# ibm-granite/dolomite-engine

Hardware: AMD Instinct MI355X
Metric: tokens/sec/node GPTDolomite-3B bf16 seq4096 padding-free (higher is better)
Workload: dtype bf16; 1 GPU; gptdolomite-3b-bf16-seq4096-paddingfree-pretrain; model=GPTDolomite-3B, global_batch=16, seq_len=4096, parallelism=dp1

## Files before the change

dolomite_engine_amd/csrc/attention.hip:

```cpp

#include "common.h"

typedef __bf16 bf16x8 __attribute__((ext_vector_type(8)));
typedef float f32x4 __attribute__((ext_vector_type(4)));

#define MFMA16(a, b, c) __builtin_amdgcn_mfma_f32_16x16x32_bf16((a), (b), (c), 0, 0, 0)

#define DOL_LOG2E 1.44269504088896340736f
#define DOL_LN2 0.69314718055994530942f

#define PI23(q) (((q) & ~12) | ((((q) >> 2) & 1) << 3) | ((((q) >> 3) & 1) << 2))

typedef __bf16 bf16x4 __attribute__((ext_vector_type(4)));


__device__ __forceinline__ bf16x8 lds_tr16_bfrag(const __bf16* img, int rowbase, int S, int d0, int lane) {
    const int g8 = (lane >> 4) * 8;
    const int jj = (lane >> 2) & 3;
    const int cc = (lane & 3) * 4;
    unsigned a0 = (unsigned)(size_t)(img + PI23(rowbase + g8 + jj) * S + d0 + cc);
    unsigned a1 = (unsigned)(size_t)(img + PI23(rowbase + g8 + 4 + jj) * S + d0 + cc);
    bf16x4 lo, hi;
    asm volatile(
        "ds_read_b64_tr_b16 %0, %2\n\t"
        "ds_read_b64_tr_b16 %1, %3\n\t"
        "s_waitcnt lgkmcnt(0)"
        : "=&v"(lo), "=&v"(hi)
        : "v"(a0), "v"(a1)
        : "memory");
    bf16x8 out;
#pragma unroll
    for (int t = 0; t < 4; ++t) { out[t] = lo[t]; out[4 + t] = hi[t]; }
    return out;
}


template <int OFF>
__device__ __forceinline__ void tr16_issue(unsigned a0, unsigned a1, bf16x4& lo, bf16x4& hi) {
    asm volatile(
        "ds_read_b64_tr_b16 %0, %2 offset:%c4\n\t"
        "ds_read_b64_tr_b16 %1, %3 offset:%c4"
        : "=&v"(lo), "=&v"(hi)
        : "v"(a0), "v"(a1), "i"(OFF)
        : "memory");
}

template <int N>
__device__ __forceinline__ void lgkm_wait2(bf16x4& a, bf16x4& b) {
    asm volatile("s_waitcnt lgkmcnt(%c2)" : "+v"(a), "+v"(b) : "i"(N));
}
template <int N>
__device__ __forceinline__ void lgkm_wait4(bf16x4& a, bf16x4& b, bf16x4& c, bf16x4& d) {
    asm volatile("s_waitcnt lgkmcnt(%c4)" : "+v"(a), "+v"(b), "+v"(c), "+v"(d) : "i"(N));
}
template <int N>
__device__ __forceinline__ void lgkm_wait8(bf16x4& a, bf16x4& b, bf16x4& c, bf16x4& d,
                                           bf16x4& e, bf16x4& f, bf16x4& g, bf16x4& h) {
    asm volatile("s_waitcnt lgkmcnt(%c8)"
                 : "+v"(a), "+v"(b), "+v"(c), "+v"(d), "+v"(e), "+v"(f), "+v"(g), "+v"(h)
                 : "i"(N));
}

__device__ __forceinline__ bf16x8 tr16_join8(bf16x4 lo, bf16x4 hi) {
    bf16x8 out;
#pragma unroll
    for (int t = 0; t < 4; ++t) { out[t] = lo[t]; out[4 + t] = hi[t]; }
    return out;
}

__device__ __forceinline__ void lgkm_drain2x8(bf16x8& a, bf16x8& b) {
    asm volatile("s_waitcnt lgkmcnt(0)" : "+v"(a), "+v"(b));
}
__device__ __forceinline__ void lgkm_drain4x8(bf16x8& a, bf16x8& b, bf16x8& c, bf16x8& d) {
    asm volatile("s_waitcnt lgkmcnt(0)" : "+v"(a), "+v"(b), "+v"(c), "+v"(d));
}

__device__ __forceinline__ bf16x8 load_bf16x8_guard(const __bf16* p, int d0, int D, bool valid) {
    const __bf16* q = (d0 < D) ? p : (p - d0);
    bool ok = valid && (d0 < D);
    bf16x8 r = *(const bf16x8*)q;
#pragma unroll
    for (int e = 0; e < 8; ++e) r[e] = ok ? r[e] : (__bf16)0.f;
    return r;
}

__device__ __forceinline__ float qwave_reduce_max(float v) {
    v = fmaxf(v, dpp_ror_f32<8>(v));
    v = fmaxf(v, dpp_ror_f32<4>(v));
    v = fmaxf(v, dpp_ror_f32<2>(v));
    v = fmaxf(v, dpp_ror_f32<1>(v));
    return v;
}
__device__ __forceinline__ float qwave_reduce_sum(float v) {
    v += dpp_ror_f32<8>(v);
    v += dpp_ror_f32<4>(v);
    v += dpp_ror_f32<2>(v);
    v += dpp_ror_f32<1>(v);
    return v;
}


__device__ __forceinline__ void xcd_remap_tile_bh(int& tile, int& b, int& h) {
    const int ntile = gridDim.x, nb = gridDim.y, nh = gridDim.z;
    const int64_t nbh = (int64_t)nb * nh;
    if (nbh % 8 != 0) return;
    int64_t raw = blockIdx.x + (int64_t)ntile * (blockIdx.y + (int64_t)nb * blockIdx.z);
    int xcd = (int)(raw % 8);
    int64_t idx = raw / 8;
    int64_t pair_local = idx / ntile;
    tile = (int)(idx % ntile);
    int64_t pair = pair_local * 8 + xcd;
    b = (int)(pair % nb);
    h = (int)(pair / nb);
}

#define DOL_DROP_CQ 0x9E3779B1u
#define DOL_DROP_CK 0x85EBCA77u
#define DOL_DROP_CH 0xC2B2AE3Du
#define DOL_DROP_M1 0x7FEB352Du
#define DOL_DROP_M2 0x846CA68Bu

__device__ __forceinline__ uint32_t drop_mix32(uint32_t x) {
    x ^= x >> 16;
    x *= DOL_DROP_M1;
    x ^= x >> 15;
    x *= DOL_DROP_M2;
    x ^= x >> 16;
    return x;
}
__device__ __forceinline__ uint32_t drop_head_word(uint32_t seed_hi, uint32_t h) {
    return drop_mix32(seed_hi ^ (h * DOL_DROP_CH));
}
__device__ __forceinline__ uint32_t drop_row_word(uint32_t seed_lo, uint32_t t_q) {
    return drop_mix32(seed_lo ^ (t_q * DOL_DROP_CQ));
}
__device__ __forceinline__ uint32_t drop_col_word(uint32_t head_word, uint32_t t_k) {
    return drop_mix32(head_word ^ (t_k * DOL_DROP_CK));
}
__device__ __forceinline__ bool drop_keep_words(uint32_t rw, uint32_t cw, uint32_t thr) {
    uint32_t x = rw ^ cw;
    x ^= x >> 16;
    x *= DOL_DROP_M1;
    x ^= x >> 15;
    x *= DOL_DROP_M2;
    return x >= thr;
}
__device__ __forceinline__ bool drop_keep(uint32_t seed_lo, uint32_t seed_hi, uint32_t h,
                                          uint32_t t_q, uint32_t t_k, uint32_t thr) {
    return drop_keep_words(drop_row_word(seed_lo, t_q),
                           drop_col_word(drop_head_word(seed_hi, h), t_k), thr);
}

static inline uint32_t drop_threshold(float p_drop) {
    return (uint32_t)((double)p_drop * 4294967296.0);
}
static inline bool drop_p_valid(float p_drop) { return p_drop >= 0.f && p_drop < 1.f; }


template <int DPAD, bool DROPOUT>
__global__ void __launch_bounds__(512, 4) fa_fwd_kernel(
    const __bf16* __restrict__ q, const __bf16* __restrict__ k, const __bf16* __restrict__ v,
    __bf16* __restrict__ o, float* __restrict__ lse,
    const int32_t* __restrict__ cu, int H, int Hkv, int D, int G,
    int64_t q_ts, int64_t q_gs, int64_t k_ts, int64_t k_hs, int64_t v_ts, int64_t v_hs,
    int64_t o_ts, int64_t T_total, float scale,
    uint32_t seed_lo, uint32_t seed_hi, uint32_t drop_thr, float drop_rp) {
    constexpr int KCH = DPAD / 32;
    constexpr int DCH = DPAD / 16;
    constexpr int SK = DPAD + 16;
    constexpr int SV = 64 + 8;

    int tile_id = blockIdx.x, b = blockIdx.y, h = blockIdx.z;
    xcd_remap_tile_bh(tile_id, b, h);
    const int s0 = __builtin_amdgcn_readfirstlane(cu[b]);
    const int L = __builtin_amdgcn_readfirstlane(cu[b + 1]) - s0;
    const int ntile_seq = (L + 127) / 128;
    if (tile_id >= ntile_seq) return;
    const int qs = (ntile_seq - 1 - tile_id) * 128;

    const int lane = threadIdx.x & 63;
    const int wave = threadIdx.x >> 6;
    const int lr = lane & 15;
    const int lg = lane >> 4;

    constexpr int NBUF = 1;
    extern __shared__ char smem_raw[];
    __bf16* Klds = (__bf16*)smem_raw;
    __bf16* Vlds = Klds + NBUF * 64 * SK;
    __bf16* Plds = Vlds + NBUF * 64 * SK;
    __bf16* Pw = Plds + wave * 16 * SV;

    const int kvh = h / G;
    const int64_t q_hoff = (int64_t)(h / G) * q_gs + (int64_t)(h % G) * D;

    const int qrow = qs + wave * 16 + lr;
    const bool qvalid = qrow < L;
    bf16x8 qf[KCH];
#pragma unroll
    for (int kc = 0; kc < KCH; ++kc) {
        int d0 = kc * 32 + lg * 8;
        const __bf16* p = q + (int64_t)(s0 + (qvalid ? qrow : 0)) * q_ts + q_hoff + d0;
        qf[kc] = load_bf16x8_guard(p, d0, D, qvalid);
    }

    float m_run[4], l_run[4];
    f32x4 o_acc[DCH];
#pragma unroll
    for (int r = 0; r < 4; ++r) { m_run[r] = -INFINITY; l_run[r] = 0.f; }
#pragma unroll
    for (int dc = 0; dc < DCH; ++dc) o_acc[dc] = {0.f, 0.f, 0.f, 0.f};

    uint32_t drop_rw[4];
    uint32_t drop_hw = 0;
    if constexpr (DROPOUT) {
        drop_hw = drop_head_word(seed_hi, (uint32_t)h);
#pragma unroll
        for (int r = 0; r < 4; ++r)
            drop_rw[r] = drop_row_word(seed_lo, (uint32_t)(s0 + qs + wave * 16 + lg * 4 + r));
    }

    const int tr_jj = (lane >> 2) & 3;
    const int tr_g8 = (lane >> 4) * 8;
    const int tr_cc = (lane & 3) * 4;
    const unsigned aV0 = (unsigned)(size_t)(Vlds + PI23(tr_g8 + tr_jj) * SK + tr_cc);
    const unsigned aV1 = (unsigned)(size_t)(Vlds + PI23(tr_g8 + 4 + tr_jj) * SK + tr_cc);

    const int kend = min(L, qs + 128);
    const int ntiles = (kend + 63) / 64;

    if (D < DPAD) {
        for (int pidx = threadIdx.x; pidx < 64 * (DPAD - D) / 8; pidx += 512) {
            int key = pidx / ((DPAD - D) / 8);
            int d0 = D + (pidx % ((DPAD - D) / 8)) * 8;
            bf16x8 z = {};
            *(bf16x8*)&Klds[key * SK + d0] = z;
            *(bf16x8*)&Vlds[PI23(key) * SK + d0] = z;
        }
    }

    int st_koff[2], st_voff[2];
    int st_klds[2], st_vlds[2];
#pragma unroll
    for (int j = 0; j < 2; ++j) {
        int pidx = (int)threadIdx.x + j * 512;
        int pp = pidx < 64 * D / 8 ? pidx : 0;
        int key = pp / (D / 8);
        int d0 = (pp % (D / 8)) * 8;
        st_koff[j] = (int)(key * k_ts + kvh * k_hs) + d0;
        st_voff[j] = (int)(key * v_ts + kvh * v_hs) + d0;
        st_klds[j] = key * SK + d0;
        st_vlds[j] = PI23(key) * SK + d0;
    }

    if (__builtin_amdgcn_readfirstlane(threadIdx.x) >= 256) __builtin_amdgcn_s_setprio(1);

    constexpr int PIECES = 64 * DPAD / 8;

    auto stage_direct = [&](int ks_, __bf16* Kw, __bf16* Vw) {
        if (ks_ + 64 <= kend) {
            const int64_t disp = (int64_t)(s0 + ks_);
#pragma unroll
            for (int j = 0; j < 2; ++j) {
                if ((int)threadIdx.x + j * 512 < 64 * D / 8) {
                    *(bf16x8*)&Kw[st_klds[j]] = *(const bf16x8*)(k + disp * k_ts + st_koff[j]);
                    *(bf16x8*)&Vw[st_vlds[j]] = *(const bf16x8*)(v + disp * v_ts + st_voff[j]);
                }
            }
        } else {
            for (int pidx = threadIdx.x; pidx < PIECES; pidx += 512) {
                int key = pidx / (DPAD / 8);
                int d0 = (pidx % (DPAD / 8)) * 8;
                bool kv_valid = (ks_ + key) < kend;
                const __bf16* kp = k + (int64_t)(s0 + (kv_valid ? ks_ + key : 0)) * k_ts + (int64_t)kvh * k_hs + d0;
                *(bf16x8*)&Kw[key * SK + d0] = load_bf16x8_guard(kp, d0, D, kv_valid);
                const __bf16* vp = v + (int64_t)(s0 + (kv_valid ? ks_ + key : 0)) * v_ts + (int64_t)kvh * v_hs + d0;
                *(bf16x8*)&Vw[PI23(key) * SK + d0] = load_bf16x8_guard(vp, d0, D, kv_valid);
            }
        }
    };

    auto compute_tile = [&](const __bf16* Kb, unsigned aV0c, unsigned aV1c, int ks) {
        f32x4 sc[4];
#pragma unroll
        for (int cb = 0; cb < 4; ++cb) {
            sc[cb] = {0.f, 0.f, 0.f, 0.f};
#pragma unroll
            for (int kc = 0; kc < KCH; ++kc) {
                bf16x8 kf = *(const bf16x8*)&Kb[(cb * 16 + lr) * SK + kc * 32 + lg * 8];
                sc[cb] = MFMA16(qf[kc], kf, sc[cb]);
            }
        }

        const float scale2 = scale * DOL_LOG2E;
        const bool edge_tile =
            !((ks + 63 <= qs + wave * 16) && (ks + 64 <= kend) && (qs + wave * 16 + 16 <= L));
        uint32_t drop_cw[4];
        if constexpr (DROPOUT) {
#pragma unroll
            for (int cb = 0; cb < 4; ++cb)
                drop_cw[cb] = drop_col_word(drop_hw, (uint32_t)(s0 + ks + cb * 16 + lr));
        }
#pragma unroll
        for (int r = 0; r < 4; ++r) {
            float pv[4];
#pragma unroll
            for (int cb = 0; cb < 4; ++cb) pv[cb] = sc[cb][r] * scale2;
            if (__builtin_amdgcn_readfirstlane(edge_tile ? 1 : 0)) {
                const int qpos = qs + wave * 16 + lg * 4 + r;
#pragma unroll
                for (int cb = 0; cb < 4; ++cb) {
                    const int kpos = ks + cb * 16 + lr;
                    if (kpos > qpos || kpos >= kend || qpos >= L) pv[cb] = -INFINITY;
                }
            }
            float rowmax = fmaxf(fmaxf(pv[0], pv[1]), fmaxf(pv[2], pv[3]));
            rowmax = qwave_reduce_max(rowmax);
            float mnew = fmaxf(m_run[r], rowmax);
            if (mnew == -INFINITY) mnew = 0.f;
            float alpha = exp2f(m_run[r] - mnew);
            float rsum = 0.f;
#pragma unroll
            for (int cb = 0; cb < 4; ++cb) {
                float e = exp2f(pv[cb] - mnew);
                float ek = e;
                if constexpr (DROPOUT)
                    ek = drop_keep_words(drop_rw[r], drop_cw[cb], drop_thr) ? e : 0.f;
                Pw[(lg * 4 + r) * SV + cb * 16 + lr] = (__bf16)ek;
                rsum += e;
            }
            rsum = qwave_reduce_sum(rsum);
            l_run[r] = l_run[r] * alpha + rsum;
            m_run[r] = mnew;
#pragma unroll
            for (int dc = 0; dc < DCH; ++dc) o_acc[dc][r] *= alpha;
        }

        {
            bf16x8 pf0 = *(const bf16x8*)&Pw[lr * SV + lg * 8];
            bf16x8 pf1 = *(const bf16x8*)&Pw[lr * SV + 32 + lg * 8];
            lgkm_drain2x8(pf0, pf1);
            __builtin_amdgcn_sched_barrier(0);
            bf16x4 vlo[3], vhi[3];
            tr16_issue<0>(aV0c, aV1c, vlo[0], vhi[0]);
            tr16_issue<((1 / DCH) * 32 * SK + (1 % DCH) * 16) * 2>(aV0c, aV1c, vlo[1], vhi[1]);
#define FWD_PV_STEP(i)                                                                                  \
    if constexpr ((i) < 2 * DCH) {                                                                      \
        constexpr int kc2_ = (i) / DCH, dc_ = (i) % DCH;                                                \
        if constexpr ((i) + 2 < 2 * DCH) {                                                              \
            constexpr int kn_ = ((i) + 2) / DCH, dn_ = ((i) + 2) % DCH;                                 \
            tr16_issue<(kn_ * 32 * SK + dn_ * 16) * 2>(aV0c, aV1c, vlo[((i) + 2) % 3], vhi[((i) + 2) % 3]); \
            lgkm_wait2<4>(vlo[(i) % 3], vhi[(i) % 3]);                                                  \
        } else if constexpr ((i) + 1 < 2 * DCH) {                                                       \
            lgkm_wait2<2>(vlo[(i) % 3], vhi[(i) % 3]);                                                  \
        } else {                                                                                        \
            lgkm_wait2<0>(vlo[(i) % 3], vhi[(i) % 3]);                                                  \
        }                                                                                               \
        o_acc[dc_] = MFMA16(kc2_ ? pf1 : pf0, tr16_join8(vlo[(i) % 3], vhi[(i) % 3]), o_acc[dc_]);      \
    }
            FWD_PV_STEP(0) FWD_PV_STEP(1) FWD_PV_STEP(2) FWD_PV_STEP(3)
            FWD_PV_STEP(4) FWD_PV_STEP(5) FWD_PV_STEP(6) FWD_PV_STEP(7)
            FWD_PV_STEP(8) FWD_PV_STEP(9) FWD_PV_STEP(10) FWD_PV_STEP(11)
            FWD_PV_STEP(12) FWD_PV_STEP(13) FWD_PV_STEP(14) FWD_PV_STEP(15)
#undef FWD_PV_STEP
            __builtin_amdgcn_sched_barrier(0);
        }
    };

    if constexpr (NBUF == 2) {
        constexpr int CH = (64 * SK * 2) / 1024;
        constexpr int NC = (2 * CH + 7) / 8;
        auto rsrcK = __builtin_amdgcn_make_buffer_rsrc(
            (void*)(k + (int64_t)s0 * k_ts + (int64_t)kvh * k_hs), 0,
            (unsigned)(((int64_t)(L - 1) * k_ts + D) * 2), 0);
        auto rsrcV = __builtin_amdgcn_make_buffer_rsrc(
            (void*)(v + (int64_t)s0 * v_ts + (int64_t)kvh * v_hs), 0,
            (unsigned)(((int64_t)(L - 1) * v_ts + D) * 2), 0);
        unsigned choff[NC];
        bool ch_is_v[NC];
#pragma unroll
        for (int i = 0; i < NC; ++i) {
            int c = wave + i * 8;
            bool isv = c >= CH;
            int cc = isv ? c - CH : c;
            int e0 = cc * 512 + lane * 8;
            int row = e0 / SK;
            int col = e0 % SK;
            int key = isv ? PI23(row) : row;
            int64_t ts = isv ? v_ts : k_ts;
            unsigned off = (unsigned)((key * ts + col) * 2);
            if (col >= D || c >= 2 * CH) off = 0x40000000u;
            choff[i] = off;
            ch_is_v[i] = isv;
        }
        const unsigned kstep2 = (unsigned)(k_ts * 2) * 64u;
        const unsigned vstep2 = (unsigned)(v_ts * 2) * 64u;

        auto stage_dma = [&](int kt_, int buf_) {
            __bf16* Kb = Klds + buf_ * 64 * SK;
            __bf16* Vb = Vlds + buf_ * 64 * SK;
#pragma unroll
            for (int i = 0; i < NC; ++i) {
                int c = wave + i * 8;
                if (c >= 2 * CH) break;
                bool isv = ch_is_v[i];
                int cc = isv ? c - CH : c;
                char* ldsp = (char*)(isv ? Vb : Kb) + cc * 1024;
                unsigned vo = choff[i] + (unsigned)kt_ * (isv ? vstep2 : kstep2);
                __builtin_amdgcn_raw_ptr_buffer_load_lds(
                    isv ? rsrcV : rsrcK,
                    (__attribute__((address_space(3))) void*)ldsp, 16, vo, 0, 0, 0);
            }
        };

        stage_dma(0, 0);
        asm volatile("s_waitcnt vmcnt(0)" ::: "memory");
        __syncthreads();
        for (int kt = 0; kt < ntiles; ++kt) {
            const int cur = kt & 1;
            if (kt + 1 < ntiles) stage_dma(kt + 1, cur ^ 1);
            compute_tile(Klds + cur * 64 * SK,
                         aV0 + (unsigned)(cur * 64 * SK * 2),
                         aV1 + (unsigned)(cur * 64 * SK * 2), kt * 64);
            asm volatile("s_waitcnt vmcnt(0)" ::: "memory");
            __syncthreads();
        }
    } else {
        for (int kt = 0; kt < ntiles; ++kt) {
            stage_direct(kt * 64, Klds, Vlds);
            __syncthreads();
            compute_tile(Klds, aV0, aV1, kt * 64);
            __syncthreads();
        }
    }

    float inv_l[4];
#pragma unroll
    for (int r = 0; r < 4; ++r) {
        inv_l[r] = (l_run[r] > 0.f) ? 1.f / l_run[r] : 0.f;
        if constexpr (DROPOUT) inv_l[r] *= drop_rp;
        const int qpos = qs + wave * 16 + lg * 4 + r;
        if (lr == 0 && qpos < L)
            lse[(int64_t)h * T_total + s0 + qpos] = (m_run[r] + log2f(l_run[r])) * DOL_LN2;
    }
#pragma unroll
    for (int dc = 0; dc < DCH; ++dc) {
#pragma unroll
        for (int r = 0; r < 4; ++r) {
            const int qpos = qs + wave * 16 + lg * 4 + r;
            const int d = dc * 16 + lr;
            if (qpos < L && d < D)
                o[(int64_t)(s0 + qpos) * o_ts + (int64_t)h * D + d] = (__bf16)(o_acc[dc][r] * inv_l[r]);
        }
    }
}

template <int DPAD, bool DROPOUT>
static int launch_fa_fwd(hipStream_t stream, const __bf16* q, const __bf16* k, const __bf16* v,
                         __bf16* o, float* lse, const int32_t* cu, int batch, int64_t T,
                         int H, int Hkv, int D, int G,
                         int64_t q_ts, int64_t q_gs, int64_t k_ts, int64_t k_hs,
                         int64_t v_ts, int64_t v_hs, int max_tiles, float scale,
                         float p_drop, uint64_t seed) {
    dim3 grid(max_tiles, batch, H), block(512);
    size_t shmem = ((size_t)(DPAD <= 96 ? 2 : 1) * 64 * (DPAD + 16) * 2 + 8 * 16 * 72) * sizeof(__bf16);
    hipLaunchKernelGGL((fa_fwd_kernel<DPAD, DROPOUT>), grid, block, shmem, stream,
                       q, k, v, o, lse, cu, H, Hkv, D, G,
                       q_ts, q_gs, k_ts, k_hs, v_ts, v_hs, (int64_t)H * D, T, scale,
                       (uint32_t)seed, (uint32_t)(seed >> 32), drop_threshold(p_drop),
                       1.f / (1.f - p_drop));
    return dol_last_error();
}

static int fa_varlen_fwd_dispatch(dolomite_stream_t stream,
                                  const void* q, const void* k, const void* v,
                                  void* o, float* lse,
                                  const int32_t* cu_seqlens, int batch, int max_seqlen, int64_t T,
                                  int H, int Hkv, int D, int G,
                                  int64_t q_tstride, int64_t q_gstride,
                                  int64_t k_tstride, int64_t k_hstride,
                                  int64_t v_tstride, int64_t v_hstride,
                                  float scale, int dtype, float p_drop, uint64_t seed) {
    if (dtype != DOLOMITE_BF16) return 9010;
    if (D > 128) return 9011;
    int max_tiles = (max_seqlen + 127) / 128;
    hipStream_t s = (hipStream_t)stream;
#define CASE(DP, DROP)                                                                               \
    return launch_fa_fwd<DP, DROP>(s, (const __bf16*)q, (const __bf16*)k, (const __bf16*)v,          \
                                   (__bf16*)o, lse, cu_seqlens, batch, T, H, Hkv, D, G, q_tstride,   \
                                   q_gstride, k_tstride, k_hstride, v_tstride, v_hstride, max_tiles, \
                                   scale, p_drop, seed)
    if (p_drop > 0.f) {
        if (D <= 32) CASE(32, true);
        if (D <= 64) CASE(64, true);
        if (D <= 96) CASE(96, true);
        CASE(128, true);
    }
    if (D <= 32) CASE(32, false);
    if (D <= 64) CASE(64, false);
    if (D <= 96) CASE(96, false);
    CASE(128, false);
#undef CASE
}

extern "C" int dolomite_fa_varlen_fwd(dolomite_stream_t stream,
                                      const void* q, const void* k, const void* v,
                                      void* o, float* lse,
                                      const int32_t* cu_seqlens, int batch, int max_seqlen, int64_t T,
                                      int H, int Hkv, int D, int G,
                                      int64_t q_tstride, int64_t q_gstride,
                                      int64_t k_tstride, int64_t k_hstride,
                                      int64_t v_tstride, int64_t v_hstride,
                                      float scale, int dtype) {
    return fa_varlen_fwd_dispatch(stream, q, k, v, o, lse, cu_seqlens, batch, max_seqlen, T,
                                  H, Hkv, D, G, q_tstride, q_gstride, k_tstride, k_hstride,
                                  v_tstride, v_hstride, scale, dtype, 0.f, 0);
}

extern "C" int dolomite_fa_varlen_fwd_dropout(dolomite_stream_t stream,
                                              const void* q, const void* k, const void* v,
                                              void* o, float* lse,
                                              const int32_t* cu_seqlens, int batch, int max_seqlen, int64_t T,
                                              int H, int Hkv, int D, int G,
                                              int64_t q_tstride, int64_t q_gstride,
                                              int64_t k_tstride, int64_t k_hstride,
                                              int64_t v_tstride, int64_t v_hstride,
                                              float scale, int dtype, float p_drop, uint64_t seed) {
    if (!drop_p_valid(p_drop)) return 9013;
    return fa_varlen_fwd_dispatch(stream, q, k, v, o, lse, cu_seqlens, batch, max_seqlen, T,
                                  H, Hkv, D, G, q_tstride, q_gstride, k_tstride, k_hstride,
                                  v_tstride, v_hstride, scale, dtype, p_drop, seed);
}


template <typename T>
__global__ void __launch_bounds__(256) fa_bwd_preprocess_kernel(
    const T* __restrict__ o, const T* __restrict__ dout, float* __restrict__ delta,
    int64_t T_total, int H, int D, int64_t o_ts, int64_t do_ts) {
    int64_t row = ((int64_t)blockIdx.x * 4) + (threadIdx.x >> 6);
    int lane = threadIdx.x & 63;
    if (row >= T_total * H) return;
    int64_t t = row / H;
    int h = (int)(row % H);
    const T* op = o + t * o_ts + (int64_t)h * D;
    const T* dp = dout + t * do_ts + (int64_t)h * D;
    float acc = 0.f;
    for (int d = lane * 2; d + 1 < D; d += 128) {
        float o0[2], d0[2];
        VecIO<T, 2>::load(op + d, o0);
        VecIO<T, 2>::load(dp + d, d0);
        acc += o0[0] * d0[0] + o0[1] * d0[1];
    }
    if (D & 1) {
        int d = D - 1;
        if (lane == 0) acc += load_as_f32(op + d) * load_as_f32(dp + d);
    }
    acc = wave_reduce_sum(acc);
    if (lane == 0) delta[(int64_t)h * T_total + t] = acc;
}

__global__ void __launch_bounds__(256) fa_bwd_preprocess_tiled(
    const __bf16* __restrict__ o, const __bf16* __restrict__ dout, float* __restrict__ delta,
    int64_t T_total, int H, int D, int TOK) {
    extern __shared__ float part[];
    const int64_t hd = (int64_t)H * D;
    const int64_t base = (int64_t)blockIdx.x * TOK * hd;
    const int64_t total = T_total * hd;
    const int np = (int)(TOK * hd / 8);
#pragma unroll 4
    for (int p = threadIdx.x; p < np; p += 256) {
        int64_t flat = base + (int64_t)p * 8;
        float acc = 0.f;
        if (flat + 8 <= total) {
            bf16x8 ov = *(const bf16x8*)(o + flat);
            bf16x8 dv = *(const bf16x8*)(dout + flat);
#pragma unroll
            for (int e = 0; e < 8; ++e) acc += (float)ov[e] * (float)dv[e];
        }
        part[p] = acc;
    }
    __syncthreads();
    const int slots = TOK * H;
    const int dp8 = D / 8;
    for (int s = threadIdx.x; s < slots; s += 256) {
        float a = 0.f;
        const float* ps = &part[s * dp8];
        for (int i = 0; i < dp8; ++i) a += ps[i];
        int tl = s / H, h = s - tl * H;
        int64_t t = (int64_t)blockIdx.x * TOK + tl;
        if (t < T_total) delta[(int64_t)h * T_total + t] = a;
    }
}

extern "C" int dolomite_fa_bwd_preprocess(dolomite_stream_t stream,
                                          const void* o, const void* dout, float* delta,
                                          int64_t T, int H, int D,
                                          int64_t o_tstride, int64_t do_tstride, int dtype) {
    const int64_t hd = (int64_t)H * D;
    int TOK = 16;
    while (TOK > 1 && TOK * hd * 4 / 8 > 65536) TOK /= 2;
    if (dtype == DOLOMITE_BF16 && D % 8 == 0 && o_tstride == hd && do_tstride == hd && T > 0 &&
        TOK * hd * 4 / 8 <= 65536) {
        dim3 grid((uint32_t)((T + TOK - 1) / TOK)), block(256);
        size_t shmem = (size_t)(TOK * hd / 8) * sizeof(float);
        hipLaunchKernelGGL((fa_bwd_preprocess_tiled), grid, block, shmem, (hipStream_t)stream,
                           (const __bf16*)o, (const __bf16*)dout, delta, T, H, D, TOK);
        return dol_last_error();
    }
    int64_t rows = T * H;
    dim3 grid((uint32_t)((rows + 3) / 4)), block(256);
    if (dtype == DOLOMITE_BF16)
        hipLaunchKernelGGL((fa_bwd_preprocess_kernel<uint16_t>), grid, block, 0, (hipStream_t)stream,
                           (const uint16_t*)o, (const uint16_t*)dout, delta, T, H, D, o_tstride, do_tstride);
    else
        hipLaunchKernelGGL((fa_bwd_preprocess_kernel<float>), grid, block, 0, (hipStream_t)stream,
                           (const float*)o, (const float*)dout, delta, T, H, D, o_tstride, do_tstride);
    return dol_last_error();
}



template <int DPAD, bool DROPOUT>
__global__ void __launch_bounds__(512, DPAD <= 96 ? 4 : 2) fa_bwd_dkv_kernel(
    const __bf16* __restrict__ q, const __bf16* __restrict__ k, const __bf16* __restrict__ v,
    const __bf16* __restrict__ dout, const float* __restrict__ lse, const float* __restrict__ delta,
    float* __restrict__ dk_acc, float* __restrict__ dv_acc,
    const int32_t* __restrict__ cu, int H, int Hkv, int D, int G,
    int64_t q_ts, int64_t q_gs, int64_t k_ts, int64_t k_hs, int64_t v_ts, int64_t v_hs,
    int64_t do_ts, int64_t T_total, float scale,
    uint32_t seed_lo, uint32_t seed_hi, uint32_t drop_thr, float drop_rp) {
    constexpr int KCH = DPAD / 32;
    constexpr int DCH = DPAD / 16;

    int tile_id = blockIdx.x, b = blockIdx.y, h = blockIdx.z;
    xcd_remap_tile_bh(tile_id, b, h);
    const int kvh = h / G;
    const int s0 = __builtin_amdgcn_readfirstlane(cu[b]);
    const int L = __builtin_amdgcn_readfirstlane(cu[b + 1]) - s0;
    const int ks = tile_id * 128;
    if (ks >= L) return;

    const int lane = threadIdx.x & 63;
    const int wave = threadIdx.x >> 6;
    const int lr = lane & 15;
    const int lg = lane >> 4;

    constexpr int SQ = DPAD + 16;
    constexpr int STS = 128 + 4;
    extern __shared__ char smem_raw[];
    __bf16* Qlds = (__bf16*)smem_raw;
    __bf16* dOl = Qlds + 64 * SQ;
    __bf16* dSTl = dOl + 64 * SQ;
    __bf16* PTl = dSTl + 64 * STS;

    const int kend = min(L, ks + 128);

    const int krow = ks + wave * 16 + lr;
    const bool kvalid = krow < kend;
    bf16x8 kfr[KCH], vfr[KCH];
#pragma unroll
    for (int kc = 0; kc < KCH; ++kc) {
        int d0 = kc * 32 + lg * 8;
        const __bf16* kp = k + (int64_t)(s0 + (kvalid ? krow : 0)) * k_ts + (int64_t)kvh * k_hs + d0;
        kfr[kc] = load_bf16x8_guard(kp, d0, D, kvalid);
        const __bf16* vp = v + (int64_t)(s0 + (kvalid ? krow : 0)) * v_ts + (int64_t)kvh * v_hs + d0;
        vfr[kc] = load_bf16x8_guard(vp, d0, D, kvalid);
    }

    f32x4 dvr[DCH], dkr[DCH];
#pragma unroll
    for (int dc = 0; dc < DCH; ++dc) {
        dvr[dc] = {0.f, 0.f, 0.f, 0.f};
        dkr[dc] = {0.f, 0.f, 0.f, 0.f};
    }

    uint32_t drop_cw[4];
    if constexpr (DROPOUT) {
        const uint32_t drop_hw = drop_head_word(seed_hi, (uint32_t)h);
#pragma unroll
        for (int r = 0; r < 4; ++r)
            drop_cw[r] = drop_col_word(drop_hw, (uint32_t)(s0 + ks + wave * 16 + lg * 4 + r));
    }

    const int tr_jj = (lane >> 2) & 3;
    const int tr_g8 = (lane >> 4) * 8;
    const int tr_cc = (lane & 3) * 4;
    const unsigned aQ0 = (unsigned)(size_t)(Qlds + PI23(tr_g8 + tr_jj) * SQ + tr_cc);
    const unsigned aQ1 = (unsigned)(size_t)(Qlds + PI23(tr_g8 + 4 + tr_jj) * SQ + tr_cc);
    const unsigned aDS0 = (unsigned)(size_t)(dSTl + PI23(tr_g8 + tr_jj) * STS + wave * 16 + tr_cc);
    const unsigned aDS1 = (unsigned)(size_t)(dSTl + PI23(tr_g8 + 4 + tr_jj) * STS + wave * 16 + tr_cc);
    constexpr int DO_IMM = 64 * SQ * 2;
    constexpr int PT_IMM = 64 * STS * 2;
    static_assert(DO_IMM + 32 * SQ * 2 + 16 * 2 < 65536, "ds offset range");
    static_assert(PT_IMM + 32 * STS * 2 + 16 * 2 < 65536, "ds offset range");

    if (__builtin_amdgcn_readfirstlane(threadIdx.x) >= 256) __builtin_amdgcn_s_setprio(1);

    const int qt0 = ks / 64;
    const int nqt = (L + 63) / 64;
    const int64_t q_hoff = (int64_t)(h / G) * q_gs + (int64_t)(h % G) * D;
    const int64_t do_hoff = (int64_t)h * D;

    if (D < DPAD) {
        for (int pidx = threadIdx.x; pidx < 64 * (DPAD - D) / 8; pidx += 512) {
            int qq = pidx / ((DPAD - D) / 8);
            int d0 = D + (pidx % ((DPAD - D) / 8)) * 8;
            bf16x8 z = {};
            *(bf16x8*)&Qlds[PI23(qq) * SQ + d0] = z;
            *(bf16x8*)&dOl[PI23(qq) * SQ + d0] = z;
        }
    }

    const unsigned st_magic = (1u << 22) / (unsigned)(D / 8) + 1;
    for (int qt = qt0; qt < nqt; ++qt) {
        const int qs = qt * 64;
        __syncthreads();
        {
            const int pieces = 64 * DPAD / 8;
            if (qs + 64 <= L) {
                for (int pidx = threadIdx.x; pidx < 64 * D / 8; pidx += 512) {
                    int qq = (int)(((unsigned)pidx * st_magic) >> 22);
                    int d0 = (pidx - qq * (D / 8)) * 8;
                    *(bf16x8*)&Qlds[PI23(qq) * SQ + d0] =
                        *(const bf16x8*)(q + (int64_t)(s0 + qs + qq) * q_ts + q_hoff + d0);
                    *(bf16x8*)&dOl[PI23(qq) * SQ + d0] =
                        *(const bf16x8*)(dout + (int64_t)(s0 + qs + qq) * do_ts + do_hoff + d0);
                }
            } else {
                for (int pidx = threadIdx.x; pidx < pieces; pidx += 512) {
                    int qq = pidx / (DPAD / 8);
                    int d0 = (pidx % (DPAD / 8)) * 8;
                    bool valid = (qs + qq) < L;
                    const __bf16* qp = q + (int64_t)(s0 + (valid ? qs + qq : 0)) * q_ts + q_hoff + d0;
                    *(bf16x8*)&Qlds[PI23(qq) * SQ + d0] = load_bf16x8_guard(qp, d0, D, valid);
                    const __bf16* dp = dout + (int64_t)(s0 + (valid ? qs + qq : 0)) * do_ts + do_hoff + d0;
                    *(bf16x8*)&dOl[PI23(qq) * SQ + d0] = load_bf16x8_guard(dp, d0, D, valid);
                }
            }
        }
        __syncthreads();

        const bool full_tile = (ks + wave * 16 + 16 <= qs + 1) && (kend == ks + 64) && (qs + 64 <= L);
#pragma unroll
        for (int cb = 0; cb < 4; ++cb) {
            f32x4 st = {0.f, 0.f, 0.f, 0.f};
            f32x4 dpt = {0.f, 0.f, 0.f, 0.f};
#pragma unroll
            for (int kc = 0; kc < KCH; ++kc) {
                int d0 = kc * 32 + lg * 8;
                bf16x8 qb = *(const bf16x8*)&Qlds[(cb * 16 + PI23(lr)) * SQ + d0];
                st = MFMA16(kfr[kc], qb, st);
                bf16x8 db = *(const bf16x8*)&dOl[(cb * 16 + PI23(lr)) * SQ + d0];
                dpt = MFMA16(vfr[kc], db, dpt);
            }
            const int qpos = qs + cb * 16 + lr;
            const bool qok = qpos < L;
            float lsev = qok ? lse[(int64_t)h * T_total + s0 + qpos] * DOL_LOG2E : 0.f;
            float delv = qok ? delta[(int64_t)h * T_total + s0 + qpos] : 0.f;
            bf16x4 pvv, dsv;
            uint32_t drop_rw = 0;
            if constexpr (DROPOUT) drop_rw = drop_row_word(seed_lo, (uint32_t)(s0 + qpos));
            if (__builtin_amdgcn_readfirstlane(full_tile ? 1 : 0)) {
#pragma unroll
                for (int r = 0; r < 4; ++r) {
                    float pv = exp2f(st[r] * (scale * DOL_LOG2E) - lsev);
                    if constexpr (DROPOUT) {
                        const bool keep = drop_keep_words(drop_rw, drop_cw[r], drop_thr);
                        pvv[r] = (__bf16)(keep ? pv : 0.f);
                        dsv[r] = (__bf16)(pv * ((keep ? dpt[r] * drop_rp : 0.f) - delv) * scale);
                    } else {
                        pvv[r] = (__bf16)pv;
                        dsv[r] = (__bf16)(pv * (dpt[r] - delv) * scale);
                    }
                }
            } else {
#pragma unroll
                for (int r = 0; r < 4; ++r) {
                    const int kpos = ks + wave * 16 + lg * 4 + r;
                    bool ok = qok && kpos < kend && kpos <= qpos;
                    float pv = ok ? exp2f(st[r] * (scale * DOL_LOG2E) - lsev) : 0.f;
                    if constexpr (DROPOUT) {
                        const bool keep = drop_keep_words(drop_rw, drop_cw[r], drop_thr);
                        float ds = ok ? pv * ((keep ? dpt[r] * drop_rp : 0.f) - delv) * scale : 0.f;
                        pvv[r] = (__bf16)(keep ? pv : 0.f);
                        dsv[r] = (__bf16)ds;
                    } else {
                        float ds = ok ? pv * (dpt[r] - delv) * scale : 0.f;
                        pvv[r] = (__bf16)pv;
                        dsv[r] = (__bf16)ds;
                    }
                }
            }
            const int srow = PI23(cb * 16 + lr) * STS + wave * 16 + lg * 4;
            *(bf16x4*)&PTl[srow] = pvv;
            *(bf16x4*)&dSTl[srow] = dsv;
        }

        {
            asm volatile("s_waitcnt lgkmcnt(0)" ::: "memory");
            __builtin_amdgcn_sched_barrier(0);
            bf16x4 a_lo[2], a_hi[2];
            tr16_issue<PT_IMM>(aDS0, aDS1, a_lo[0], a_hi[0]);
            tr16_issue<PT_IMM + 32 * STS * 2>(aDS0, aDS1, a_lo[1], a_hi[1]);
            bf16x4 blo[3], bhi[3];
            tr16_issue<DO_IMM>(aQ0, aQ1, blo[0], bhi[0]);
            tr16_issue<DO_IMM + ((1 / DCH) * 32 * SQ + (1 % DCH) * 16) * 2>(aQ0, aQ1, blo[1], bhi[1]);
            lgkm_wait4<4>(a_lo[0], a_hi[0], a_lo[1], a_hi[1]);
            bf16x8 af0 = tr16_join8(a_lo[0], a_hi[0]);
            bf16x8 af1 = tr16_join8(a_lo[1], a_hi[1]);
#define DKV_HALF(i, IMM, ACC, AF0, AF1)                                                                 \
    if constexpr ((i) < 2 * DCH) {                                                                      \
        constexpr int kc2_ = (i) / DCH, dc_ = (i) % DCH;                                                \
        if constexpr ((i) + 2 < 2 * DCH) {                                                              \
            constexpr int kn_ = ((i) + 2) / DCH, dn_ = ((i) + 2) % DCH;                                 \
            tr16_issue<(kn_ * 32 * SQ + dn_ * 16) * 2 + (IMM)>(aQ0, aQ1, blo[((i) + 2) % 3], bhi[((i) + 2) % 3]); \
            lgkm_wait2<4>(blo[(i) % 3], bhi[(i) % 3]);                                                  \
        } else if constexpr ((i) + 1 < 2 * DCH) {                                                       \
            lgkm_wait2<2>(blo[(i) % 3], bhi[(i) % 3]);                                                  \
        } else {                                                                                        \
            lgkm_wait2<0>(blo[(i) % 3], bhi[(i) % 3]);                                                  \
        }                                                                                               \
        ACC[dc_] = MFMA16(kc2_ ? (AF1) : (AF0), tr16_join8(blo[(i) % 3], bhi[(i) % 3]), ACC[dc_]);      \
    }
#define DKV_A(i) DKV_HALF(i, DO_IMM, dvr, af0, af1)
            DKV_A(0) DKV_A(1) DKV_A(2) DKV_A(3)
            DKV_A(4) DKV_A(5) DKV_A(6) DKV_A(7)
            DKV_A(8) DKV_A(9) DKV_A(10) DKV_A(11)
            DKV_A(12) DKV_A(13) DKV_A(14) DKV_A(15)
#undef DKV_A
            tr16_issue<0>(aDS0, aDS1, a_lo[0], a_hi[0]);
            tr16_issue<32 * STS * 2>(aDS0, aDS1, a_lo[1], a_hi[1]);
            tr16_issue<0>(aQ0, aQ1, blo[0], bhi[0]);
            tr16_issue<((1 / DCH) * 32 * SQ + (1 % DCH) * 16) * 2>(aQ0, aQ1, blo[1], bhi[1]);
            lgkm_wait4<4>(a_lo[0], a_hi[0], a_lo[1], a_hi[1]);
            af0 = tr16_join8(a_lo[0], a_hi[0]);
            af1 = tr16_join8(a_lo[1], a_hi[1]);
#define DKV_B(i) DKV_HALF(i, 0, dkr, af0, af1)
            DKV_B(0) DKV_B(1) DKV_B(2) DKV_B(3)
            DKV_B(4) DKV_B(5) DKV_B(6) DKV_B(7)
            DKV_B(8) DKV_B(9) DKV_B(10) DKV_B(11)
            DKV_B(12) DKV_B(13) DKV_B(14) DKV_B(15)
#undef DKV_B
#undef DKV_HALF
            __builtin_amdgcn_sched_barrier(0);
        }
    }

#pragma unroll
    for (int dc = 0; dc < DCH; ++dc) {
#pragma unroll
        for (int r = 0; r < 4; ++r) {
            const int kpos = ks + wave * 16 + lg * 4 + r;
            const int d = dc * 16 + lr;
            if (kpos < kend && d < D) {
                int64_t idx = ((int64_t)(s0 + kpos) * H + h) * D + d;
                __builtin_nontemporal_store(dkr[dc][r], &dk_acc[idx]);
                if constexpr (DROPOUT)
                    __builtin_nontemporal_store(dvr[dc][r] * drop_rp, &dv_acc[idx]);
                else
                    __builtin_nontemporal_store(dvr[dc][r], &dv_acc[idx]);
            }
        }
    }
}

template <int DPAD, bool DROPOUT>
__global__ void __launch_bounds__(512, (DROPOUT && DPAD > 96) ? 2 : 4) fa_bwd_dq_kernel(
    const __bf16* __restrict__ q, const __bf16* __restrict__ k, const __bf16* __restrict__ v,
    const __bf16* __restrict__ dout, const float* __restrict__ lse, const float* __restrict__ delta,
    __bf16* __restrict__ dqkv_q,
    const int32_t* __restrict__ cu, int H, int Hkv, int D, int G,
    int64_t q_ts, int64_t q_gs, int64_t k_ts, int64_t k_hs, int64_t v_ts, int64_t v_hs,
    int64_t do_ts, int64_t T_total, float scale,
    uint32_t seed_lo, uint32_t seed_hi, uint32_t drop_thr, float drop_rp) {
    constexpr int KCH = DPAD / 32;
    constexpr int DCH = DPAD / 16;
    constexpr int ST = 64 + 8;

    int tile_id = blockIdx.x, b = blockIdx.y, h = blockIdx.z;
    xcd_remap_tile_bh(tile_id, b, h);
    const int kvh = h / G;
    const int s0 = __builtin_amdgcn_readfirstlane(cu[b]);
    const int L = __builtin_amdgcn_readfirstlane(cu[b + 1]) - s0;
    const int ntile_seq = (L + 127) / 128;
    if (tile_id >= ntile_seq) return;
    const int qs = (ntile_seq - 1 - tile_id) * 128;

    const int lane = threadIdx.x & 63;
    const int wave = threadIdx.x >> 6;
    const int lr = lane & 15;
    const int lg = lane >> 4;

    constexpr int SQ = DPAD + 16;
    extern __shared__ char smem_raw[];
    __bf16* Klds = (__bf16*)smem_raw;
    __bf16* Vlds = Klds + 64 * SQ;
    __bf16* dSl = Vlds + 64 * SQ;
    __bf16* dSw = dSl + wave * 16 * ST;

    const int64_t q_hoff = (int64_t)(h / G) * q_gs + (int64_t)(h % G) * D;
    const int64_t do_hoff = (int64_t)h * D;

    const int tr_jj = (lane >> 2) & 3;
    const int tr_g8 = (lane >> 4) * 8;
    const int tr_cc = (lane & 3) * 4;
    const unsigned aK0 = (unsigned)(size_t)(Klds + PI23(tr_g8 + tr_jj) * SQ + tr_cc);
    const unsigned aK1 = (unsigned)(size_t)(Klds + PI23(tr_g8 + 4 + tr_jj) * SQ + tr_cc);

    const int qrow = qs + wave * 16 + lr;
    const bool qvalid = qrow < L;
    bf16x8 qfr[KCH], dfr[KCH];
#pragma unroll
    for (int kc = 0; kc < KCH; ++kc) {
        int d0 = kc * 32 + lg * 8;
        const __bf16* qp = q + (int64_t)(s0 + (qvalid ? qrow : 0)) * q_ts + q_hoff + d0;
        qfr[kc] = load_bf16x8_guard(qp, d0, D, qvalid);
        const __bf16* dp = dout + (int64_t)(s0 + (qvalid ? qrow : 0)) * do_ts + do_hoff + d0;
        dfr[kc] = load_bf16x8_guard(dp, d0, D, qvalid);
    }

    float lsev[4], delv[4];
#pragma unroll
    for (int r = 0; r < 4; ++r) {
        const int qp_ = qs + wave * 16 + lg * 4 + r;
        bool ok = qp_ < L;
        lsev[r] = ok ? lse[(int64_t)h * T_total + s0 + qp_] * DOL_LOG2E : 0.f;
        delv[r] = ok ? delta[(int64_t)h * T_total + s0 + qp_] : 0.f;
    }

    f32x4 dq[DCH];
#pragma unroll
    for (int dc = 0; dc < DCH; ++dc) dq[dc] = {0.f, 0.f, 0.f, 0.f};

    uint32_t drop_rw[4];
    uint32_t drop_hw = 0;
    if constexpr (DROPOUT) {
        drop_hw = drop_head_word(seed_hi, (uint32_t)h);
#pragma unroll
        for (int r = 0; r < 4; ++r)
            drop_rw[r] = drop_row_word(seed_lo, (uint32_t)(s0 + qs + wave * 16 + lg * 4 + r));
    }

    if (D < DPAD) {
        for (int pidx = threadIdx.x; pidx < 64 * (DPAD - D) / 8; pidx += 512) {
            int key = pidx / ((DPAD - D) / 8);
            int d0 = D + (pidx % ((DPAD - D) / 8)) * 8;
            bf16x8 z = {};
            *(bf16x8*)&Klds[PI23(key) * SQ + d0] = z;
            *(bf16x8*)&Vlds[key * SQ + d0] = z;
        }
    }

    int st_koff[2], st_voff[2];
    int st_klds[2], st_vlds[2];
#pragma unroll
    for (int j = 0; j < 2; ++j) {
        int pidx = (int)threadIdx.x + j * 512;
        int pp = pidx < 64 * D / 8 ? pidx : 0;
        int key = pp / (D / 8);
        int d0 = (pp % (D / 8)) * 8;
        st_koff[j] = (int)(key * k_ts + kvh * k_hs) + d0;
        st_voff[j] = (int)(key * v_ts + kvh * v_hs) + d0;
        st_klds[j] = PI23(key) * SQ + d0;
        st_vlds[j] = key * SQ + d0;
    }

    const int kend_total = min(L, qs + 128);
    const int nkt = (kend_total + 63) / 64;

    if (__builtin_amdgcn_readfirstlane(threadIdx.x) >= 256) __builtin_amdgcn_s_setprio(1);

    for (int kt = 0; kt < nkt; ++kt) {
        const int ks = kt * 64;
        __syncthreads();
        {
            const int pieces = 64 * DPAD / 8;
            if (ks + 64 <= kend_total) {
                const int64_t disp = (int64_t)(s0 + ks);
#pragma unroll
                for (int j = 0; j < 2; ++j) {
                    if ((int)threadIdx.x + j * 512 < 64 * D / 8) {
                        *(bf16x8*)&Klds[st_klds[j]] = *(const bf16x8*)(k + disp * k_ts + st_koff[j]);
                        *(bf16x8*)&Vlds[st_vlds[j]] = *(const bf16x8*)(v + disp * v_ts + st_voff[j]);
                    }
                }
            } else {
                for (int pidx = threadIdx.x; pidx < pieces; pidx += 512) {
                    int key = pidx / (DPAD / 8);
                    int d0 = (pidx % (DPAD / 8)) * 8;
                    bool valid = (ks + key) < kend_total;
                    const __bf16* kp = k + (int64_t)(s0 + (valid ? ks + key : 0)) * k_ts + (int64_t)kvh * k_hs + d0;
                    *(bf16x8*)&Klds[PI23(key) * SQ + d0] = load_bf16x8_guard(kp, d0, D, valid);
                    const __bf16* vp = v + (int64_t)(s0 + (valid ? ks + key : 0)) * v_ts + (int64_t)kvh * v_hs + d0;
                    *(bf16x8*)&Vlds[key * SQ + d0] = load_bf16x8_guard(vp, d0, D, valid);
                }
            }
        }
        __syncthreads();

        const bool full_tile = (ks + 64 <= qs + wave * 16 + 1) && (ks + 64 <= kend_total) && (qs + wave * 16 + 16 <= L);
#pragma unroll
        for (int cb = 0; cb < 4; ++cb) {
            f32x4 sc = {0.f, 0.f, 0.f, 0.f};
            f32x4 dp = {0.f, 0.f, 0.f, 0.f};
#pragma unroll
            for (int kc = 0; kc < KCH; ++kc) {
                int d0 = kc * 32 + lg * 8;
                bf16x8 kb = *(const bf16x8*)&Klds[(cb * 16 + PI23(lr)) * SQ + d0];
                sc = MFMA16(qfr[kc], kb, sc);
                bf16x8 vb = *(const bf16x8*)&Vlds[(cb * 16 + lr) * SQ + d0];
                dp = MFMA16(dfr[kc], vb, dp);
            }
            uint32_t drop_cw = 0;
            if constexpr (DROPOUT) drop_cw = drop_col_word(drop_hw, (uint32_t)(s0 + ks + cb * 16 + lr));
            if (__builtin_amdgcn_readfirstlane(full_tile ? 1 : 0)) {
#pragma unroll
                for (int r = 0; r < 4; ++r) {
                    float pv = exp2f(sc[r] * (scale * DOL_LOG2E) - lsev[r]);
                    float dpm = dp[r];
                    if constexpr (DROPOUT)
                        dpm = drop_keep_words(drop_rw[r], drop_cw, drop_thr) ? dp[r] * drop_rp : 0.f;
                    dSw[(lg * 4 + r) * ST + cb * 16 + lr] = (__bf16)(pv * (dpm - delv[r]) * scale);
                }
            } else {
#pragma unroll
                for (int r = 0; r < 4; ++r) {
                    const int qpos = qs + wave * 16 + lg * 4 + r;
                    const int kpos = ks + cb * 16 + lr;
                    bool ok = qpos < L && kpos < kend_total && kpos <= qpos;
                    float pv = ok ? exp2f(sc[r] * (scale * DOL_LOG2E) - lsev[r]) : 0.f;
                    float dpm = dp[r];
                    if constexpr (DROPOUT)
                        dpm = drop_keep_words(drop_rw[r], drop_cw, drop_thr) ? dp[r] * drop_rp : 0.f;
                    float ds = ok ? pv * (dpm - delv[r]) * scale : 0.f;
                    dSw[(lg * 4 + r) * ST + cb * 16 + lr] = (__bf16)ds;
                }
            }
        }

        {
            bf16x8 dsf0 = *(const bf16x8*)&dSw[lr * ST + lg * 8];
            bf16x8 dsf1 = *(const bf16x8*)&dSw[lr * ST + 32 + lg * 8];
            lgkm_drain2x8(dsf0, dsf1);
            __builtin_amdgcn_sched_barrier(0);
            bf16x4 klo[4], khi[4];
            tr16_issue<0>(aK0, aK1, klo[0], khi[0]);
            tr16_issue<((1 / DCH) * 32 * SQ + (1 % DCH) * 16) * 2>(aK0, aK1, klo[1], khi[1]);
            tr16_issue<((2 / DCH) * 32 * SQ + (2 % DCH) * 16) * 2>(aK0, aK1, klo[2], khi[2]);
#define DQ_STEP(i)                                                                                      \
    if constexpr ((i) < 2 * DCH) {                                                                      \
        constexpr int kc2_ = (i) / DCH, dc_ = (i) % DCH;                                                \
        if constexpr ((i) + 3 < 2 * DCH) {                                                              \
            constexpr int kn_ = ((i) + 3) / DCH, dn_ = ((i) + 3) % DCH;                                 \
            tr16_issue<(kn_ * 32 * SQ + dn_ * 16) * 2>(aK0, aK1, klo[((i) + 3) % 4], khi[((i) + 3) % 4]); \
            lgkm_wait2<6>(klo[(i) % 4], khi[(i) % 4]);                                                  \
        } else if constexpr ((i) + 2 < 2 * DCH) {                                                       \
            lgkm_wait2<4>(klo[(i) % 4], khi[(i) % 4]);                                                  \
        } else if constexpr ((i) + 1 < 2 * DCH) {                                                       \
            lgkm_wait2<2>(klo[(i) % 4], khi[(i) % 4]);                                                  \
        } else {                                                                                        \
            lgkm_wait2<0>(klo[(i) % 4], khi[(i) % 4]);                                                  \
        }                                                                                               \
        dq[dc_] = MFMA16(kc2_ ? dsf1 : dsf0, tr16_join8(klo[(i) % 4], khi[(i) % 4]), dq[dc_]);          \
    }
            DQ_STEP(0) DQ_STEP(1) DQ_STEP(2) DQ_STEP(3)
            DQ_STEP(4) DQ_STEP(5) DQ_STEP(6) DQ_STEP(7)
            DQ_STEP(8) DQ_STEP(9) DQ_STEP(10) DQ_STEP(11)
            DQ_STEP(12) DQ_STEP(13) DQ_STEP(14) DQ_STEP(15)
#undef DQ_STEP
            __builtin_amdgcn_sched_barrier(0);
        }
    }

#pragma unroll
    for (int dc = 0; dc < DCH; ++dc) {
#pragma unroll
        for (int r = 0; r < 4; ++r) {
            const int qpos = qs + wave * 16 + lg * 4 + r;
            const int d = dc * 16 + lr;
            if (qpos < L && d < D)
                dqkv_q[(int64_t)(s0 + qpos) * q_ts + q_hoff + d] = (__bf16)dq[dc][r];
        }
    }
}

template <int DPAD, bool DROPOUT>
static int launch_fa_bwd(hipStream_t stream, const __bf16* q, const __bf16* k, const __bf16* v,
                         const __bf16* dout, const float* lse, const float* delta,
                         __bf16* dqkv_q, float* dk_acc, float* dv_acc,
                         const int32_t* cu, int batch, int64_t T, int H, int Hkv, int D, int G,
                         int64_t q_ts, int64_t q_gs, int64_t k_ts, int64_t k_hs,
                         int64_t v_ts, int64_t v_hs, int64_t do_ts, int max_tiles, float scale,
                         float p_drop, uint64_t seed) {
    constexpr int ST = 64 + 8;
    dim3 block(512);
    dim3 grid(max_tiles, batch, H);
    constexpr int SQ = DPAD + 16;
    const uint32_t seed_lo = (uint32_t)seed, seed_hi = (uint32_t)(seed >> 32);
    const uint32_t thr = drop_threshold(p_drop);
    const float rp = 1.f / (1.f - p_drop);
    size_t shmem_dkv = (size_t)(64 * (128 + 4) * 2 + 64 * SQ * 2) * sizeof(__bf16);
    hipLaunchKernelGGL((fa_bwd_dkv_kernel<DPAD, DROPOUT>), grid, block, shmem_dkv, stream,
                       q, k, v, dout, lse, delta, dk_acc, dv_acc, cu, H, Hkv, D, G,
                       q_ts, q_gs, k_ts, k_hs, v_ts, v_hs, do_ts, T, scale,
                       seed_lo, seed_hi, thr, rp);
    int err = dol_last_error();
    if (err) return err;
    size_t shmem_dq = (size_t)(64 * SQ * 2 + 8 * 16 * ST) * sizeof(__bf16);
    hipLaunchKernelGGL((fa_bwd_dq_kernel<DPAD, DROPOUT>), grid, block, shmem_dq, stream,
                       q, k, v, dout, lse, delta, dqkv_q, cu, H, Hkv, D, G,
                       q_ts, q_gs, k_ts, k_hs, v_ts, v_hs, do_ts, T, scale,
                       seed_lo, seed_hi, thr, rp);
    return dol_last_error();
}

static int fa_varlen_bwd_dispatch(dolomite_stream_t stream,
                                  const void* q, const void* k, const void* v,
                                  const void* dout, const float* lse,
                                  const float* delta, void* dqkv_q, float* dk_acc, float* dv_acc,
                                  const int32_t* cu_seqlens, int batch, int max_seqlen, int64_t T,
                                  int H, int Hkv, int D, int G,
                                  int64_t q_tstride, int64_t q_gstride,
                                  int64_t k_tstride, int64_t k_hstride,
                                  int64_t v_tstride, int64_t v_hstride,
                                  int64_t do_tstride,
                                  float scale, int dtype, float p_drop, uint64_t seed) {
    if (dtype != DOLOMITE_BF16) return 9010;
    if (D > 128) return 9011;
    int max_tiles = (max_seqlen + 127) / 128;
    hipStream_t s = (hipStream_t)stream;
#define CASE(DP, DROP)                                                                                  \
    return launch_fa_bwd<DP, DROP>(s, (const __bf16*)q, (const __bf16*)k, (const __bf16*)v,             \
                                   (const __bf16*)dout, lse, delta, (__bf16*)dqkv_q, dk_acc, dv_acc,    \
                                   cu_seqlens, batch, T, H, Hkv, D, G, q_tstride, q_gstride, k_tstride, \
                                   k_hstride, v_tstride, v_hstride, do_tstride, max_tiles, scale,       \
                                   p_drop, seed)
    if (p_drop > 0.f) {
        if (D <= 32) CASE(32, true);
        if (D <= 64) CASE(64, true);
        if (D <= 96) CASE(96, true);
        CASE(128, true);
    }
    if (D <= 32) CASE(32, false);
    if (D <= 64) CASE(64, false);
    if (D <= 96) CASE(96, false);
    CASE(128, false);
#undef CASE
}

extern "C" int dolomite_fa_varlen_bwd(dolomite_stream_t stream,
                                      const void* q, const void* k, const void* v,
                                      const void* dout, const float* lse,
                                      const float* delta, void* dqkv_q, float* dk_acc, float* dv_acc,
                                      const int32_t* cu_seqlens, int batch, int max_seqlen, int64_t T,
                                      int H, int Hkv, int D, int G,
                                      int64_t q_tstride, int64_t q_gstride,
                                      int64_t k_tstride, int64_t k_hstride,
                                      int64_t v_tstride, int64_t v_hstride,
                                      int64_t do_tstride,
                                      float scale, int dtype) {
    return fa_varlen_bwd_dispatch(stream, q, k, v, dout, lse, delta, dqkv_q, dk_acc, dv_acc,
                                  cu_seqlens, batch, max_seqlen, T, H, Hkv, D, G,
                                  q_tstride, q_gstride, k_tstride, k_hstride, v_tstride, v_hstride,
                                  do_tstride, scale, dtype, 0.f, 0);
}

extern "C" int dolomite_fa_varlen_bwd_dropout(dolomite_stream_t stream,
                                              const void* q, const void* k, const void* v,
                                              const void* dout, const float* lse,
                                              const float* delta, void* dqkv_q, float* dk_acc, float* dv_acc,
                                              const int32_t* cu_seqlens, int batch, int max_seqlen, int64_t T,
                                              int H, int Hkv, int D, int G,
                                              int64_t q_tstride, int64_t q_gstride,
                                              int64_t k_tstride, int64_t k_hstride,
                                              int64_t v_tstride, int64_t v_hstride,
                                              int64_t do_tstride,
                                              float scale, int dtype, float p_drop, uint64_t seed) {
    if (!drop_p_valid(p_drop)) return 9013;
    return fa_varlen_bwd_dispatch(stream, q, k, v, dout, lse, delta, dqkv_q, dk_acc, dv_acc,
                                  cu_seqlens, batch, max_seqlen, T, H, Hkv, D, G,
                                  q_tstride, q_gstride, k_tstride, k_hstride, v_tstride, v_hstride,
                                  do_tstride, scale, dtype, p_drop, seed);
}

__global__ void __launch_bounds__(256) fa_dropout_mask_probe_kernel(
    uint8_t* __restrict__ out, uint32_t seed_lo, uint32_t seed_hi, uint32_t thr,
    int64_t total, int64_t tq0, int nq, int64_t tk0, int nk) {
    const int64_t idx = (int64_t)blockIdx.x * 256 + threadIdx.x;
    if (idx >= total) return;
    const int j = (int)(idx % nk);
    const int64_t hi = idx / nk;
    const int i = (int)(hi % nq);
    const uint32_t h = (uint32_t)(hi / nq);
    out[idx] = drop_keep(seed_lo, seed_hi, h, (uint32_t)(tq0 + i), (uint32_t)(tk0 + j), thr) ? 1 : 0;
}

extern "C" int dolomite_fa_dropout_mask_probe(dolomite_stream_t stream, uint8_t* out,
                                              uint64_t seed, float p_drop, int H,
                                              int64_t tq0, int nq, int64_t tk0, int nk) {
    if (!drop_p_valid(p_drop)) return 9013;
    if (H < 0 || nq < 0 || nk < 0) return 9014;
    const int64_t total = (int64_t)H * nq * nk;
    if (total == 0) return 0;
    const int64_t nblocks = (total + 255) / 256;
    if (nblocks > 0x7fffffff) return 9014;
    hipLaunchKernelGGL(fa_dropout_mask_probe_kernel, dim3((uint32_t)nblocks), dim3(256), 0,
                       (hipStream_t)stream, out, (uint32_t)seed, (uint32_t)(seed >> 32),
                       drop_threshold(p_drop), total, tq0, nq, tk0, nk);
    return dol_last_error();
}


template <typename T>
__global__ void __launch_bounds__(256) fa_grad_finalize_kernel(
    const float* __restrict__ dk_acc, const float* __restrict__ dv_acc,
    T* __restrict__ dqkv, int64_t total_kv,
    int Hkv, int D, int G, int64_t row_ts, int64_t k_off, int64_t kv_hs, int64_t v_off) {
    int64_t quad = (int64_t)blockIdx.x * blockDim.x + threadIdx.x;
    int64_t total_q4 = total_kv / 4;
    bool is_v = quad >= total_q4;
    if (is_v) quad -= total_q4;
    if (quad >= total_q4) return;
    int64_t kidx = quad * 4;
    int64_t t = kidx / ((int64_t)Hkv * D);
    int rem = (int)(kidx % ((int64_t)Hkv * D));
    int j = rem / D;
    int d = rem % D;
    const float* src = is_v ? dv_acc : dk_acc;
    int64_t base = ((t * Hkv + j) * (int64_t)G) * D + d;
    f4_t acc = {0.f, 0.f, 0.f, 0.f};
    for (int g = 0; g < G; ++g) {
        f4_t v4 = __builtin_nontemporal_load((const f4_t*)&src[base + (int64_t)g * D]);
        acc += v4;
    }
    T* out = &dqkv[t * row_ts + (is_v ? v_off : k_off) + (int64_t)j * kv_hs + d];
#pragma unroll
    for (int e = 0; e < 4; ++e) store_from_f32(out + e, acc[e]);
}

extern "C" int dolomite_fa_grad_finalize(dolomite_stream_t stream,
                                         const float* dk_acc, const float* dv_acc,
                                         void* dqkv, int64_t T, int Hkv, int D, int G,
                                         int64_t row_tstride,
                                         int64_t k_off, int64_t kv_hstride, int64_t v_off, int dtype) {
    int64_t total_kv = T * (int64_t)Hkv * D;
    if (D % 4 != 0) return 9012;
    int64_t total = 2 * (total_kv / 4);
    if (total == 0) return 0;
    dim3 grid((uint32_t)((total + 255) / 256)), block(256);
    if (dtype == DOLOMITE_BF16)
        hipLaunchKernelGGL((fa_grad_finalize_kernel<uint16_t>), grid, block, 0, (hipStream_t)stream,
                           dk_acc, dv_acc, (uint16_t*)dqkv, total_kv,
                           Hkv, D, G, row_tstride, k_off, kv_hstride, v_off);
    else
        hipLaunchKernelGGL((fa_grad_finalize_kernel<float>), grid, block, 0, (hipStream_t)stream,
                           dk_acc, dv_acc, (float*)dqkv, total_kv,
                           Hkv, D, G, row_tstride, k_off, kv_hstride, v_off);
    return dol_last_error();
}


typedef __bf16 bf16x4p __attribute__((ext_vector_type(4)));
__global__ void __launch_bounds__(64) tr16_probe_kernel(float* out) {
    __shared__ __bf16 s[256];
    const int lane = threadIdx.x & 63;
    for (int i = threadIdx.x; i < 256; i += 64) s[i] = (__bf16)(float)i;
    __syncthreads();
    const unsigned base = (unsigned)(size_t)(__bf16*)s;
    unsigned addrs[3] = {
        base + (unsigned)((lane >> 4) * 128),
        base + (unsigned)(lane * 8),
        base + (unsigned)(((lane & 15) * 2) + ((lane >> 4) * 128)),
    };
#pragma unroll
    for (int v = 0; v < 3; ++v) {
        bf16x4p r;
        asm volatile("ds_read_b64_tr_b16 %0, %1\n\ts_waitcnt lgkmcnt(0)"
                     : "=v"(r)
                     : "v"(addrs[v])
                     : "memory");
#pragma unroll
        for (int j = 0; j < 4; ++j) out[(v * 64 + lane) * 4 + j] = (float)r[j];
    }
}

extern "C" int dolomite_tr16_probe(dolomite_stream_t stream, float* out) {
    hipLaunchKernelGGL(tr16_probe_kernel, dim3(1), dim3(64), 0, (hipStream_t)stream, out);
    return dol_last_error();
}

__global__ void __launch_bounds__(64) tr16_bfrag_probe_kernel(
    const __bf16* src, float* out, int cols, int S, int rowbase, int d0) {
    extern __shared__ char smem_raw[];
    __bf16* img = (__bf16*)smem_raw;
    const int lane = threadIdx.x & 63;
    for (int i = threadIdx.x; i < 64 * (cols / 8); i += 64) {
        int row = i / (cols / 8), c8 = (i % (cols / 8)) * 8;
        *(bf16x8*)&img[PI23(row) * S + c8] = *(const bf16x8*)&src[row * cols + c8];
    }
    __syncthreads();
    bf16x8 f = lds_tr16_bfrag(img, rowbase, S, d0, lane);
#pragma unroll
    for (int e = 0; e < 8; ++e) out[lane * 8 + e] = (float)f[e];
}

extern "C" int dolomite_tr16_bfrag_probe(dolomite_stream_t stream, const void* src, float* out,
                                         int cols, int S, int rowbase, int d0) {
    size_t shmem = (size_t)64 * S * sizeof(__bf16);
    hipLaunchKernelGGL(tr16_bfrag_probe_kernel, dim3(1), dim3(64), shmem, (hipStream_t)stream,
                       (const __bf16*)src, out, cols, S, rowbase, d0);
    return dol_last_error();
}

__global__ void __launch_bounds__(64) mfma_probe_kernel(const __bf16* A, const __bf16* B, float* C) {
    int lane = threadIdx.x & 63;
    int lr = lane & 15, lg = lane >> 4;
    bf16x8 a, b;
#pragma unroll
    for (int e = 0; e < 8; ++e) {
        a[e] = A[lr * 32 + lg * 8 + e];
        b[e] = B[(lg * 8 + e) * 16 + lr];
    }
    f32x4 c = {0.f, 0.f, 0.f, 0.f};
    c = MFMA16(a, b, c);
#pragma unroll
    for (int r = 0; r < 4; ++r) C[(lg * 4 + r) * 16 + lr] = c[r];
}

extern "C" int dolomite_mfma_probe(dolomite_stream_t stream, const void* A, const void* B, float* C) {
    hipLaunchKernelGGL(mfma_probe_kernel, dim3(1), dim3(64), 0, (hipStream_t)stream,
                       (const __bf16*)A, (const __bf16*)B, C);
    return dol_last_error();
}
```

tools_lds_sim.py:

```python

from collections import defaultdict

G128_READ = [
    [0, 1, 2, 3, 12, 13, 14, 15, 20, 21, 22, 23, 24, 25, 26, 27],
    [4, 5, 6, 7, 8, 9, 10, 11, 16, 17, 18, 19, 28, 29, 30, 31],
    [32, 33, 34, 35, 44, 45, 46, 47, 52, 53, 54, 55, 56, 57, 58, 59],
    [36, 37, 38, 39, 40, 41, 42, 43, 48, 49, 50, 51, 60, 61, 62, 63],
]
G128_WRITE = [list(range(i * 8, i * 8 + 8)) for i in range(8)]
G32 = [list(range(0, 32)), list(range(32, 64))]


def cycles(addrs_bytes, groups, ndwords, bankmod):
    total = 0
    for grp in groups:
        banks = defaultdict(set)
        for lane in grp:
            a = addrs_bytes.get(lane)
            if a is None:
                continue
            for d in range(ndwords):
                dw = a // 4 + d
                banks[dw % bankmod].add(dw)
        if banks:
            total += max(len(v) for v in banks.values())
    ideal = sum(1 for grp in groups if any(addrs_bytes.get(l) is not None for l in grp))
    return total, ideal


def read128(addrs):
    return cycles(addrs, G128_READ, 4, 64)


def write128(addrs):
    return cycles(addrs, G128_WRITE, 4, 32)


def write16(addrs):
    return cycles(addrs, G32, 1, 32)


def report(name, pairs):
    c = sum(p[0] for p in pairs)
    i = sum(p[1] for p in pairs)
    print(f"  {name:42s} cycles={c:5d} ideal={i:5d} factor={c / max(i, 1):.2f}")
    return c, i


def SWZ(row, col, ST):
    return row * ST + ((((col >> 3) ^ ((row >> 3) & 7)) << 3) | (col & 7))


def lane_split(l):
    return l & 15, l >> 4


def main():
    DPAD = 96
    ST = 72
    SQ = DPAD + 8
    SK = DPAD + 8
    SV = 72

    print("== fa_bwd_dkv ==")
    tot = [0, 0]

    def acc(name, pairs):
        c, i = report(name, pairs)
        tot[0] += c
        tot[1] += i

    for base in (0, 512):
        addrs = {}
        addrsT = [dict() for _ in range(8)]
        for l in range(64):
            pidx = base + l
            if pidx >= 768:
                continue
            qq = pidx // (DPAD // 8)
            d0 = (pidx % (DPAD // 8)) * 8
            addrs[l] = (qq * SQ + d0) * 2
            for e in range(8):
                addrsT[e][l] = SWZ(d0 + e, qq, ST) * 2
        acc(f"stage b128 write Qlds (piece base {base})", [write128(addrs)])
        acc(f"stage 8x b16 scatter QTl (base {base})", [write16(a) for a in addrsT])

    pairs = []
    for cb in range(4):
        for kc in range(DPAD // 32):
            addrs = {}
            for l in range(64):
                lr, lg = lane_split(l)
                addrs[l] = ((cb * 16 + lr) * SQ + kc * 32 + lg * 8) * 2
            pairs.append(read128(addrs))
    acc("S^T/dP^T B-frag reads Qlds (x2 for dOl)", pairs)

    pairs = []
    for cb in range(4):
        for r in range(4):
            addrs = {}
            for l in range(64):
                lr, lg = lane_split(l)
                addrs[l] = ((0 * 16 + lg * 4 + r) * ST + cb * 16 + lr) * 2
            pairs.append(write16(addrs))
    acc("P^T strip b16 writes (x2 for dS^T)", pairs)

    pairs = []
    for kc2 in range(2):
        addrs = {}
        for l in range(64):
            lr, lg = lane_split(l)
            addrs[l] = ((0 * 16 + lr) * ST + kc2 * 32 + lg * 8) * 2
        pairs.append(read128(addrs))
    acc("P^T/dS^T A-frag reads (x2)", pairs)

    pairs = []
    for kc2 in range(2):
        for dc in range(DPAD // 16):
            addrs = {}
            for l in range(64):
                lr, lg = lane_split(l)
                addrs[l] = SWZ(dc * 16 + lr, kc2 * 32 + lg * 8, ST) * 2
            pairs.append(read128(addrs))
    acc("dOT/QT swizzled B-frag reads (x2)", pairs)

    print(f"  TOTAL factor (sampled instrs) = {tot[0] / tot[1]:.3f}")

    print("== fa_bwd_dq ==")
    tot = [0, 0]
    print("  (patterns identical to dkv rows)")

    print("== fa_fwd ==")
    tot = [0, 0]
    print("  (patterns identical to dkv rows, SV=SK strides)")


if __name__ == "__main__":
    main()
```

Baseline: 47790 tokens/s.

## Keep P and dS in registers by transposing MFMA operands in attention kernels

Swaps the MFMA operand order so the score tile is produced transposed. Each lane then owns one query row and can feed P (forward) or dS (dQ backward) straight from registers into the PV/dSK MFMA, instead of bouncing them through a per-wave LDS strip. Row max and row sum reductions become permlane16/32 swaps, the O rescale is skipped when alpha is 1 across the wave, and output stores become bf16x4 vector writes. Dropout column hashes are precomputed once per tile into LDS. The unused double-buffer DMA path and the PI23 row permutation are removed, which changes the tr16 read addressing and carries a risk of LDS bank conflicts.

```diff
diff --git a/dolomite_engine_amd/csrc/attention.hip b/dolomite_engine_amd/csrc/attention.hip
--- a/dolomite_engine_amd/csrc/attention.hip
+++ b/dolomite_engine_amd/csrc/attention.hip
@@ -3,6 +3,7 @@
 
 typedef __bf16 bf16x8 __attribute__((ext_vector_type(8)));
 typedef float f32x4 __attribute__((ext_vector_type(4)));
+typedef uint32_t u32x4 __attribute__((ext_vector_type(4)));
 
 #define MFMA16(a, b, c) __builtin_amdgcn_mfma_f32_16x16x32_bf16((a), (b), (c), 0, 0, 0)
 
@@ -68,13 +69,6 @@
     return out;
 }
 
-__device__ __forceinline__ void lgkm_drain2x8(bf16x8& a, bf16x8& b) {
-    asm volatile("s_waitcnt lgkmcnt(0)" : "+v"(a), "+v"(b));
-}
-__device__ __forceinline__ void lgkm_drain4x8(bf16x8& a, bf16x8& b, bf16x8& c, bf16x8& d) {
-    asm volatile("s_waitcnt lgkmcnt(0)" : "+v"(a), "+v"(b), "+v"(c), "+v"(d));
-}
-
 __device__ __forceinline__ bf16x8 load_bf16x8_guard(const __bf16* p, int d0, int D, bool valid) {
     const __bf16* q = (d0 < D) ? p : (p - d0);
     bool ok = valid && (d0 < D);
@@ -83,22 +77,6 @@
     for (int e = 0; e < 8; ++e) r[e] = ok ? r[e] : (__bf16)0.f;
     return r;
 }
-
-__device__ __forceinline__ float qwave_reduce_max(float v) {
-    v = fmaxf(v, dpp_ror_f32<8>(v));
-    v = fmaxf(v, dpp_ror_f32<4>(v));
-    v = fmaxf(v, dpp_ror_f32<2>(v));
-    v = fmaxf(v, dpp_ror_f32<1>(v));
-    return v;
-}
-__device__ __forceinline__ float qwave_reduce_sum(float v) {
-    v += dpp_ror_f32<8>(v);
-    v += dpp_ror_f32<4>(v);
-    v += dpp_ror_f32<2>(v);
-    v += dpp_ror_f32<1>(v);
-    return v;
-}
-
 
 __device__ __forceinline__ void xcd_remap_tile_bh(int& tile, int& b, int& h) {
     const int ntile = gridDim.x, nb = gridDim.y, nh = gridDim.z;
@@ -157,6 +135,37 @@
 static inline bool drop_p_valid(float p_drop) { return p_drop >= 0.f && p_drop < 1.f; }
 
 
+template <int DPAD>
+struct FaKvLds {
+    static constexpr int S = DPAD + 16;
+    static constexpr size_t image_bytes = (size_t)2 * 64 * S * sizeof(__bf16);
+    static constexpr size_t bytes(bool dropout) {
+        return image_bytes + (dropout ? 64 * sizeof(uint32_t) : 0);
+    }
+};
+
+__device__ __forceinline__ void fa_tr16_perm_bases(const __bf16* img, int S, int lane,
+                                                   unsigned& a0, unsigned& a1) {
+    const int row = (lane >> 4) * 4 + ((lane >> 2) & 3);
+    const int cc = (lane & 3) * 4;
+    a0 = (unsigned)(size_t)(img + row * S + cc);
+    a1 = (unsigned)(size_t)(img + (16 + row) * S + cc);
+}
+
+__device__ __forceinline__ float qgroup_reduce_max(float v) {
+    auto a = __builtin_amdgcn_permlane16_swap(__float_as_uint(v), __float_as_uint(v), false, false);
+    v = fmaxf(__uint_as_float(a[0]), __uint_as_float(a[1]));
+    auto b = __builtin_amdgcn_permlane32_swap(__float_as_uint(v), __float_as_uint(v), false, false);
+    return fmaxf(__uint_as_float(b[0]), __uint_as_float(b[1]));
+}
+__device__ __forceinline__ float qgroup_reduce_sum(float v) {
+    auto a = __builtin_amdgcn_permlane16_swap(__float_as_uint(v), __float_as_uint(v), false, false);
+    v = __uint_as_float(a[0]) + __uint_as_float(a[1]);
+    auto b = __builtin_amdgcn_permlane32_swap(__float_as_uint(v), __float_as_uint(v), false, false);
+    return __uint_as_float(b[0]) + __uint_as_float(b[1]);
+}
+
+
 template <int DPAD, bool DROPOUT>
 __global__ void __launch_bounds__(512, 4) fa_fwd_kernel(
     const __bf16* __restrict__ q, const __bf16* __restrict__ k, const __bf16* __restrict__ v,
@@ -167,8 +176,7 @@
     uint32_t seed_lo, uint32_t seed_hi, uint32_t drop_thr, float drop_rp) {
     constexpr int KCH = DPAD / 32;
     constexpr int DCH = DPAD / 16;
-    constexpr int SK = DPAD + 16;
-    constexpr int SV = 64 + 8;
+    constexpr int SK = FaKvLds<DPAD>::S;
 
     int tile_id = blockIdx.x, b = blockIdx.y, h = blockIdx.z;
     xcd_remap_tile_bh(tile_id, b, h);
@@ -183,12 +191,10 @@
     const int lr = lane & 15;
     const int lg = lane >> 4;
 
-    constexpr int NBUF = 1;
     extern __shared__ char smem_raw[];
     __bf16* Klds = (__bf16*)smem_raw;
-    __bf16* Vlds = Klds + NBUF * 64 * SK;
-    __bf16* Plds = Vlds + NBUF * 64 * SK;
-    __bf16* Pw = Plds + wave * 16 * SV;
+    __bf16* Vlds = Klds + 64 * SK;
+    uint32_t* Cw = (uint32_t*)(Vlds + 64 * SK);
 
     const int kvh = h / G;
     const int64_t q_hoff = (int64_t)(h / G) * q_gs + (int64_t)(h % G) * D;
@@ -203,27 +209,20 @@
         qf[kc] = load_bf16x8_guard(p, d0, D, qvalid);
     }
 
-    float m_run[4], l_run[4];
+    float m_run = -INFINITY, l_run = 0.f;
     f32x4 o_acc[DCH];
 #pragma unroll
-    for (int r = 0; r < 4; ++r) { m_run[r] = -INFINITY; l_run[r] = 0.f; }
-#pragma unroll
     for (int dc = 0; dc < DCH; ++dc) o_acc[dc] = {0.f, 0.f, 0.f, 0.f};
 
-    uint32_t drop_rw[4];
+    uint32_t drop_rw = 0;
     uint32_t drop_hw = 0;
     if constexpr (DROPOUT) {
         drop_hw = drop_head_word(seed_hi, (uint32_t)h);
-#pragma unroll
-        for (int r = 0; r < 4; ++r)
-            drop_rw[r] = drop_row_word(seed_lo, (uint32_t)(s0 + qs + wave * 16 + lg * 4 + r));
-    }
-
-    const int tr_jj = (lane >> 2) & 3;
-    const int tr_g8 = (lane >> 4) * 8;
-    const int tr_cc = (lane & 3) * 4;
-    const unsigned aV0 = (unsigned)(size_t)(Vlds + PI23(tr_g8 + tr_jj) * SK + tr_cc);
-    const unsigned aV1 = (unsigned)(size_t)(Vlds + PI23(tr_g8 + 4 + tr_jj) * SK + tr_cc);
+        drop_rw = drop_row_word(seed_lo, (uint32_t)(s0 + qrow));
+    }
+
+    unsigned aV0, aV1;
+    fa_tr16_perm_bases(Vlds, SK, lane, aV0, aV1);
 
     const int kend = min(L, qs + 128);
     const int ntiles = (kend + 63) / 64;
@@ -234,7 +233,7 @@
             int d0 = D + (pidx % ((DPAD - D) / 8)) * 8;
             bf16x8 z = {};
             *(bf16x8*)&Klds[key * SK + d0] = z;
-            *(bf16x8*)&Vlds[PI23(key) * SK + d0] = z;
+            *(bf16x8*)&Vlds[key * SK + d0] = z;
         }
     }
 
@@ -249,7 +248,7 @@
         st_koff[j] = (int)(key * k_ts + kvh * k_hs) + d0;
         st_voff[j] = (int)(key * v_ts + kvh * v_hs) + d0;
         st_klds[j] = key * SK + d0;
-        st_vlds[j] = PI23(key) * SK + d0;
+        st_vlds[j] = key * SK + d0;
     }
 
     if (__builtin_amdgcn_readfirstlane(threadIdx.x) >= 256) __builtin_amdgcn_s_setprio(1);
@@ -274,10 +273,12 @@
                 const __bf16* kp = k + (int64_t)(s0 + (kv_valid ? ks_ + key : 0)) * k_ts + (int64_t)kvh * k_hs + d0;
                 *(bf16x8*)&Kw[key * SK + d0] = load_bf16x8_guard(kp, d0, D, kv_valid);
                 const __bf16* vp = v + (int64_t)(s0 + (kv_valid ? ks_ + key : 0)) * v_ts + (int64_t)kvh * v_hs + d0;
-                *(bf16x8*)&Vw[PI23(key) * SK + d0] = load_bf16x8_guard(vp, d0, D, kv_valid);
+                *(bf16x8*)&Vw[key * SK + d0] = load_bf16x8_guard(vp, d0, D, kv_valid);
             }
         }
     };
+
+    const float scale2 = scale * DOL_LOG2E;
 
     auto compute_tile = [&](const __bf16* Kb, unsigned aV0c, unsigned aV1c, int ks) {
         f32x4 sc[4];
@@ -287,58 +288,54 @@
 #pragma unroll
             for (int kc = 0; kc < KCH; ++kc) {
                 bf16x8 kf = *(const bf16x8*)&Kb[(cb * 16 + lr) * SK + kc * 32 + lg * 8];
-                sc[cb] = MFMA16(qf[kc], kf, sc[cb]);
+                sc[cb] = MFMA16(kf, qf[kc], sc[cb]);
             }
         }
 
-        const float scale2 = scale * DOL_LOG2E;
         const bool edge_tile =
             !((ks + 63 <= qs + wave * 16) && (ks + 64 <= kend) && (qs + wave * 16 + 16 <= L));
-        uint32_t drop_cw[4];
-        if constexpr (DROPOUT) {
-#pragma unroll
-            for (int cb = 0; cb < 4; ++cb)
-                drop_cw[cb] = drop_col_word(drop_hw, (uint32_t)(s0 + ks + cb * 16 + lr));
-        }
-#pragma unroll
-        for (int r = 0; r < 4; ++r) {
-            float pv[4];
-#pragma unroll
-            for (int cb = 0; cb < 4; ++cb) pv[cb] = sc[cb][r] * scale2;
-            if (__builtin_amdgcn_readfirstlane(edge_tile ? 1 : 0)) {
-                const int qpos = qs + wave * 16 + lg * 4 + r;
-#pragma unroll
-                for (int cb = 0; cb < 4; ++cb) {
-                    const int kpos = ks + cb * 16 + lr;
-                    if (kpos > qpos || kpos >= kend || qpos >= L) pv[cb] = -INFINITY;
+        if (__builtin_amdgcn_readfirstlane(edge_tile ? 1 : 0)) {
+#pragma unroll
+            for (int cb = 0; cb < 4; ++cb) {
+#pragma unroll
+                for (int x = 0; x < 4; ++x) {
+                    const int kpos = ks + cb * 16 + lg * 4 + x;
+                    if (kpos > qrow || kpos >= kend || qrow >= L) sc[cb][x] = -INFINITY;
                 }
             }
-            float rowmax = fmaxf(fmaxf(pv[0], pv[1]), fmaxf(pv[2], pv[3]));
-            rowmax = qwave_reduce_max(rowmax);
-            float mnew = fmaxf(m_run[r], rowmax);
-            if (mnew == -INFINITY) mnew = 0.f;
-            float alpha = exp2f(m_run[r] - mnew);
-            float rsum = 0.f;
-#pragma unroll
-            for (int cb = 0; cb < 4; ++cb) {
-                float e = exp2f(pv[cb] - mnew);
+        }
+        float mx[4];
+#pragma unroll
+        for (int cb = 0; cb < 4; ++cb)
+            mx[cb] = fmaxf(fmaxf(sc[cb][0], sc[cb][1]), fmaxf(sc[cb][2], sc[cb][3]));
+        const float rowmax = qgroup_reduce_max(fmaxf(fmaxf(mx[0], mx[1]), fmaxf(mx[2], mx[3])));
+        float mnew = fmaxf(m_run, rowmax * scale2);
+        if (mnew == -INFINITY) mnew = 0.f;
+        const float alpha = exp2f(m_run - mnew);
+        m_run = mnew;
+
+        bf16x8 pf[2];
+        float rsum = 0.f;
+#pragma unroll
+        for (int cb = 0; cb < 4; ++cb) {
+            u32x4 cw = {};
+            if constexpr (DROPOUT) cw = *(const u32x4*)&Cw[cb * 16 + lg * 4];
+#pragma unroll
+            for (int x = 0; x < 4; ++x) {
+                const float e = exp2f(fmaf(sc[cb][x], scale2, -mnew));
                 float ek = e;
-                if constexpr (DROPOUT)
-                    ek = drop_keep_words(drop_rw[r], drop_cw[cb], drop_thr) ? e : 0.f;
-                Pw[(lg * 4 + r) * SV + cb * 16 + lr] = (__bf16)ek;
+                if constexpr (DROPOUT) ek = drop_keep_words(drop_rw, cw[x], drop_thr) ? e : 0.f;
+                pf[cb >> 1][(cb & 1) * 4 + x] = (__bf16)ek;
                 rsum += e;
             }
-            rsum = qwave_reduce_sum(rsum);
-            l_run[r] = l_run[r] * alpha + rsum;
-            m_run[r] = mnew;
-#pragma unroll
-            for (int dc = 0; dc < DCH; ++dc) o_acc[dc][r] *= alpha;
+        }
+        l_run = l_run * alpha + rsum;
+        if (!__all(alpha == 1.0f)) {
+#pragma unroll
+            for (int dc = 0; dc < DCH; ++dc) o_acc[dc] *= alpha;
         }
 
         {
-            bf16x8 pf0 = *(const bf16x8*)&Pw[lr * SV + lg * 8];
-            bf16x8 pf1 = *(const bf16x8*)&Pw[lr * SV + 32 + lg * 8];
-            lgkm_drain2x8(pf0, pf1);
             __builtin_amdgcn_sched_barrier(0);
             bf16x4 vlo[3], vhi[3];
             tr16_issue<0>(aV0c, aV1c, vlo[0], vhi[0]);
@@ -355,7 +352,7 @@
         } else {                                                                                        \
             lgkm_wait2<0>(vlo[(i) % 3], vhi[(i) % 3]);                                                  \
         }                                                                                               \
-        o_acc[dc_] = MFMA16(kc2_ ? pf1 : pf0, tr16_join8(vlo[(i) % 3], vhi[(i) % 3]), o_acc[dc_]);      \
+        o_acc[dc_] = MFMA16(tr16_join8(vlo[(i) % 3], vhi[(i) % 3]), pf[kc2_], o_acc[dc_]);              \
     }
             FWD_PV_STEP(0) FWD_PV_STEP(1) FWD_PV_STEP(2) FWD_PV_STEP(3)
             FWD_PV_STEP(4) FWD_PV_STEP(5) FWD_PV_STEP(6) FWD_PV_STEP(7)
@@ -366,91 +363,30 @@
         }
     };
 
-    if constexpr (NBUF == 2) {
-        constexpr int CH = (64 * SK * 2) / 1024;
-        constexpr int NC = (2 * CH + 7) / 8;
-        auto rsrcK = __builtin_amdgcn_make_buffer_rsrc(
-            (void*)(k + (int64_t)s0 * k_ts + (int64_t)kvh * k_hs), 0,
-            (unsigned)(((int64_t)(L - 1) * k_ts + D) * 2), 0);
-        auto rsrcV = __builtin_amdgcn_make_buffer_rsrc(
-            (void*)(v + (int64_t)s0 * v_ts + (int64_t)kvh * v_hs), 0,
-            (unsigned)(((int64_t)(L - 1) * v_ts + D) * 2), 0);
-        unsigned choff[NC];
-        bool ch_is_v[NC];
-#pragma unroll
-        for (int i = 0; i < NC; ++i) {
-            int c = wave + i * 8;
-            bool isv = c >= CH;
-            int cc = isv ? c - CH : c;
-            int e0 = cc * 512 + lane * 8;
-            int row = e0 / SK;
-            int col = e0 % SK;
-            int key = isv ? PI23(row) : row;
-            int64_t ts = isv ? v_ts : k_ts;
-            unsigned off = (unsigned)((key * ts + col) * 2);
-            if (col >= D || c >= 2 * CH) off = 0x40000000u;
-            choff[i] = off;
-            ch_is_v[i] = isv;
-        }
-        const unsigned kstep2 = (unsigned)(k_ts * 2) * 64u;
-        const unsigned vstep2 = (unsigned)(v_ts * 2) * 64u;
-
-        auto stage_dma = [&](int kt_, int buf_) {
-            __bf16* Kb = Klds + buf_ * 64 * SK;
-            __bf16* Vb = Vlds + buf_ * 64 * SK;
-#pragma unroll
-            for (int i = 0; i < NC; ++i) {
-                int c = wave + i * 8;
-                if (c >= 2 * CH) break;
-                bool isv = ch_is_v[i];
-                int cc = isv ? c - CH : c;
-                char* ldsp = (char*)(isv ? Vb : Kb) + cc * 1024;
-                unsigned vo = choff[i] + (unsigned)kt_ * (isv ? vstep2 : kstep2);
-                __builtin_amdgcn_raw_ptr_buffer_load_lds(
-                    isv ? rsrcV : rsrcK,
-                    (__attribute__((address_space(3))) void*)ldsp, 16, vo, 0, 0, 0);
-            }
-        };
-
-        stage_dma(0, 0);
-        asm volatile("s_waitcnt vmcnt(0)" ::: "memory");
+    for (int kt = 0; kt < ntiles; ++kt) {
+        stage_direct(kt * 64, Klds, Vlds);
+        if constexpr (DROPOUT) {
+            if (__builtin_amdgcn_readfirstlane(threadIdx.x) < 64)
+                Cw[lane] = drop_col_word(drop_hw, (uint32_t)(s0 + kt * 64 + lane));
+        }
         __syncthreads();
-        for (int kt = 0; kt < ntiles; ++kt) {
-            const int cur = kt & 1;
-            if (kt + 1 < ntiles) stage_dma(kt + 1, cur ^ 1);
-            compute_tile(Klds + cur * 64 * SK,
-                         aV0 + (unsigned)(cur * 64 * SK * 2),
-                         aV1 + (unsigned)(cur * 64 * SK * 2), kt * 64);
-            asm volatile("s_waitcnt vmcnt(0)" ::: "memory");
-            __syncthreads();
-        }
-    } else {
-        for (int kt = 0; kt < ntiles; ++kt) {
-            stage_direct(kt * 64, Klds, Vlds);
-            __syncthreads();
-            compute_tile(Klds, aV0, aV1, kt * 64);
-            __syncthreads();
-        }
-    }
-
-    float inv_l[4];
-#pragma unroll
-    for (int r = 0; r < 4; ++r) {
-        inv_l[r] = (l_run[r] > 0.f) ? 1.f / l_run[r] : 0.f;
-        if constexpr (DROPOUT) inv_l[r] *= drop_rp;
-        const int qpos = qs + wave * 16 + lg * 4 + r;
-        if (lr == 0 && qpos < L)
-            lse[(int64_t)h * T_total + s0 + qpos] = (m_run[r] + log2f(l_run[r])) * DOL_LN2;
-    }
+        compute_tile(Klds, aV0, aV1, kt * 64);
+        __syncthreads();
+    }
+
+    const float l_row = qgroup_reduce_sum(l_run);
+    float inv_l = (l_row > 0.f) ? 1.f / l_row : 0.f;
+    if constexpr (DROPOUT) inv_l *= drop_rp;
+    if (lg == 0 && qvalid)
+        lse[(int64_t)h * T_total + s0 + qrow] = (m_run + log2f(l_row)) * DOL_LN2;
+    __bf16* orow = o + (int64_t)(s0 + (qvalid ? qrow : 0)) * o_ts + (int64_t)h * D;
 #pragma unroll
     for (int dc = 0; dc < DCH; ++dc) {
-#pragma unroll
-        for (int r = 0; r < 4; ++r) {
-            const int qpos = qs + wave * 16 + lg * 4 + r;
-            const int d = dc * 16 + lr;
-            if (qpos < L && d < D)
-                o[(int64_t)(s0 + qpos) * o_ts + (int64_t)h * D + d] = (__bf16)(o_acc[dc][r] * inv_l[r]);
-        }
+        const int d0 = dc * 16 + lg * 4;
+        bf16x4 ov;
+#pragma unroll
+        for (int x = 0; x < 4; ++x) ov[x] = (__bf16)(o_acc[dc][x] * inv_l);
+        if (qvalid && d0 < D) *(bf16x4*)&orow[d0] = ov;
     }
 }
 
@@ -462,8 +398,7 @@
                          int64_t v_ts, int64_t v_hs, int max_tiles, float scale,
                          float p_drop, uint64_t seed) {
     dim3 grid(max_tiles, batch, H), block(512);
-    size_t shmem = ((size_t)(DPAD <= 96 ? 2 : 1) * 64 * (DPAD + 16) * 2 + 8 * 16 * 72) * sizeof(__bf16);
-    hipLaunchKernelGGL((fa_fwd_kernel<DPAD, DROPOUT>), grid, block, shmem, stream,
+    hipLaunchKernelGGL((fa_fwd_kernel<DPAD, DROPOUT>), grid, block, FaKvLds<DPAD>::bytes(DROPOUT), stream,
                        q, k, v, o, lse, cu, H, Hkv, D, G,
                        q_ts, q_gs, k_ts, k_hs, v_ts, v_hs, (int64_t)H * D, T, scale,
                        (uint32_t)seed, (uint32_t)(seed >> 32), drop_threshold(p_drop),
@@ -482,6 +417,7 @@
                                   float scale, int dtype, float p_drop, uint64_t seed) {
     if (dtype != DOLOMITE_BF16) return 9010;
     if (D > 128) return 9011;
+    if (!(scale > 0.f)) return 9015;
     int max_tiles = (max_seqlen + 127) / 128;
     hipStream_t s = (hipStream_t)stream;
 #define CASE(DP, DROP)                                                                               \
@@ -874,7 +810,6 @@
     uint32_t seed_lo, uint32_t seed_hi, uint32_t drop_thr, float drop_rp) {
     constexpr int KCH = DPAD / 32;
     constexpr int DCH = DPAD / 16;
-    constexpr int ST = 64 + 8;
 
     int tile_id = blockIdx.x, b = blockIdx.y, h = blockIdx.z;
     xcd_remap_tile_bh(tile_id, b, h);
@@ -890,21 +825,17 @@
     const int lr = lane & 15;
     const int lg = lane >> 4;
 
-    constexpr int SQ = DPAD + 16;
+    constexpr int SQ = FaKvLds<DPAD>::S;
     extern __shared__ char smem_raw[];
     __bf16* Klds = (__bf16*)smem_raw;
     __bf16* Vlds = Klds + 64 * SQ;
-    __bf16* dSl = Vlds + 64 * SQ;
-    __bf16* dSw = dSl + wave * 16 * ST;
+    uint32_t* Cw = (uint32_t*)(Vlds + 64 * SQ);
 
     const int64_t q_hoff = (int64_t)(h / G) * q_gs + (int64_t)(h % G) * D;
     const int64_t do_hoff = (int64_t)h * D;
 
-    const int tr_jj = (lane >> 2) & 3;
-    const int tr_g8 = (lane >> 4) * 8;
-    const int tr_cc = (lane & 3) * 4;
-    const unsigned aK0 = (unsigned)(size_t)(Klds + PI23(tr_g8 + tr_jj) * SQ + tr_cc);
-    const unsigned aK1 = (unsigned)(size_t)(Klds + PI23(tr_g8 + 4 + tr_jj) * SQ + tr_cc);
+    unsigned aK0, aK1;
+    fa_tr16_perm_bases(Klds, SQ, lane, aK0, aK1);
 
     const int qrow = qs + wave * 16 + lr;
     const bool qvalid = qrow < L;
@@ -918,26 +849,19 @@
         dfr[kc] = load_bf16x8_guard(dp, d0, D, qvalid);
     }
 
-    float lsev[4], delv[4];
-#pragma unroll
-    for (int r = 0; r < 4; ++r) {
-        const int qp_ = qs + wave * 16 + lg * 4 + r;
-        bool ok = qp_ < L;
-        lsev[r] = ok ? lse[(int64_t)h * T_total + s0 + qp_] * DOL_LOG2E : 0.f;
-        delv[r] = ok ? delta[(int64_t)h * T_total + s0 + qp_] : 0.f;
-    }
+    const float lsev = qvalid ? lse[(int64_t)h * T_total + s0 + qrow] * DOL_LOG2E : 0.f;
+    const float delv = qvalid ? delta[(int64_t)h * T_total + s0 + qrow] : 0.f;
+    const float scale2 = scale * DOL_LOG2E;
 
     f32x4 dq[DCH];
 #pragma unroll
     for (int dc = 0; dc < DCH; ++dc) dq[dc] = {0.f, 0.f, 0.f, 0.f};
 
-    uint32_t drop_rw[4];
+    uint32_t drop_rw = 0;
     uint32_t drop_hw = 0;
     if constexpr (DROPOUT) {
         drop_hw = drop_head_word(seed_hi, (uint32_t)h);
-#pragma unroll
-        for (int r = 0; r < 4; ++r)
-            drop_rw[r] = drop_row_word(seed_lo, (uint32_t)(s0 + qs + wave * 16 + lg * 4 + r));
+        drop_rw = drop_row_word(seed_lo, (uint32_t)(s0 + qrow));
     }
 
     if (D < DPAD) {
@@ -945,7 +869,7 @@
             int key = pidx / ((DPAD - D) / 8);
             int d0 = D + (pidx % ((DPAD - D) / 8)) * 8;
             bf16x8 z = {};
-            *(bf16x8*)&Klds[PI23(key) * SQ + d0] = z;
+            *(bf16x8*)&Klds[key * SQ + d0] = z;
             *(bf16x8*)&Vlds[key * SQ + d0] = z;
         }
     }
@@ -960,7 +884,7 @@
         int d0 = (pp % (D / 8)) * 8;
         st_koff[j] = (int)(key * k_ts + kvh * k_hs) + d0;
         st_voff[j] = (int)(key * v_ts + kvh * v_hs) + d0;
-        st_klds[j] = PI23(key) * SQ + d0;
+        st_klds[j] = key * SQ + d0;
         st_vlds[j] = key * SQ + d0;
     }
 
@@ -989,15 +913,20 @@
                     int d0 = (pidx % (DPAD / 8)) * 8;
                     bool valid = (ks + key) < kend_total;
                     const __bf16* kp = k + (int64_t)(s0 + (valid ? ks + key : 0)) * k_ts + (int64_t)kvh * k_hs + d0;
-                    *(bf16x8*)&Klds[PI23(key) * SQ + d0] = load_bf16x8_guard(kp, d0, D, valid);
+                    *(bf16x8*)&Klds[key * SQ + d0] = load_bf16x8_guard(kp, d0, D, valid);
                     const __bf16* vp = v + (int64_t)(s0 + (valid ? ks + key : 0)) * v_ts + (int64_t)kvh * v_hs + d0;
                     *(bf16x8*)&Vlds[key * SQ + d0] = load_bf16x8_guard(vp, d0, D, valid);
                 }
             }
+            if constexpr (DROPOUT) {
+                if (__builtin_amdgcn_readfirstlane(threadIdx.x) < 64)
+                    Cw[lane] = drop_col_word(drop_hw, (uint32_t)(s0 + ks + lane));
+            }
         }
         __syncthreads();
 
         const bool full_tile = (ks + 64 <= qs + wave * 16 + 1) && (ks + 64 <= kend_total) && (qs + wave * 16 + 16 <= L);
+        bf16x8 dsf[2];
 #pragma unroll
         for (int cb = 0; cb < 4; ++cb) {
             f32x4 sc = {0.f, 0.f, 0.f, 0.f};
@@ -1005,42 +934,38 @@
 #pragma unroll
             for (int kc = 0; kc < KCH; ++kc) {
                 int d0 = kc * 32 + lg * 8;
-                bf16x8 kb = *(const bf16x8*)&Klds[(cb * 16 + PI23(lr)) * SQ + d0];
-                sc = MFMA16(qfr[kc], kb, sc);
+                bf16x8 kb = *(const bf16x8*)&Klds[(cb * 16 + lr) * SQ + d0];
+                sc = MFMA16(kb, qfr[kc], sc);
                 bf16x8 vb = *(const bf16x8*)&Vlds[(cb * 16 + lr) * SQ + d0];
-                dp = MFMA16(dfr[kc], vb, dp);
+                dp = MFMA16(vb, dfr[kc], dp);
             }
-            uint32_t drop_cw = 0;
-            if constexpr (DROPOUT) drop_cw = drop_col_word(drop_hw, (uint32_t)(s0 + ks + cb * 16 + lr));
+            u32x4 cw = {};
+            if constexpr (DROPOUT) cw = *(const u32x4*)&Cw[cb * 16 + lg * 4];
             if (__builtin_amdgcn_readfirstlane(full_tile ? 1 : 0)) {
 #pragma unroll
-                for (int r = 0; r < 4; ++r) {
-                    float pv = exp2f(sc[r] * (scale * DOL_LOG2E) - lsev[r]);
-                    float dpm = dp[r];
+                for (int x = 0; x < 4; ++x) {
+                    float pv = exp2f(fmaf(sc[x], scale2, -lsev));
+                    float dpm = dp[x];
                     if constexpr (DROPOUT)
-                        dpm = drop_keep_words(drop_rw[r], drop_cw, drop_thr) ? dp[r] * drop_rp : 0.f;
-                    dSw[(lg * 4 + r) * ST + cb * 16 + lr] = (__bf16)(pv * (dpm - delv[r]) * scale);
+                        dpm = drop_keep_words(drop_rw, cw[x], drop_thr) ? dp[x] * drop_rp : 0.f;
+                    dsf[cb >> 1][(cb & 1) * 4 + x] = (__bf16)(pv * (dpm - delv) * scale);
                 }
             } else {
 #pragma unroll
-                for (int r = 0; r < 4; ++r) {
-                    const int qpos = qs + wave * 16 + lg * 4 + r;
-                    const int kpos = ks + cb * 16 + lr;
-                    bool ok = qpos < L && kpos < kend_total && kpos <= qpos;
-                    float pv = ok ? exp2f(sc[r] * (scale * DOL_LOG2E) - lsev[r]) : 0.f;
-                    float dpm = dp[r];
+                for (int x = 0; x < 4; ++x) {
+                    const int kpos = ks + cb * 16 + lg * 4 + x;
+                    bool ok = qvalid && kpos < kend_total && kpos <= qrow;
+                    float pv = ok ? exp2f(fmaf(sc[x], scale2, -lsev)) : 0.f;
+                    float dpm = dp[x];
                     if constexpr (DROPOUT)
-                        dpm = drop_keep_words(drop_rw[r], drop_cw, drop_thr) ? dp[r] * drop_rp : 0.f;
-                    float ds = ok ? pv * (dpm - delv[r]) * scale : 0.f;
-                    dSw[(lg * 4 + r) * ST + cb * 16 + lr] = (__bf16)ds;
+                        dpm = drop_keep_words(drop_rw, cw[x], drop_thr) ? dp[x] * drop_rp : 0.f;
+                    float ds = ok ? pv * (dpm - delv) * scale : 0.f;
+                    dsf[cb >> 1][(cb & 1) * 4 + x] = (__bf16)ds;
                 }
             }
         }
 
         {
-            bf16x8 dsf0 = *(const bf16x8*)&dSw[lr * ST + lg * 8];
-            bf16x8 dsf1 = *(const bf16x8*)&dSw[lr * ST + 32 + lg * 8];
-            lgkm_drain2x8(dsf0, dsf1);
             __builtin_amdgcn_sched_barrier(0);
             bf16x4 klo[4], khi[4];
             tr16_issue<0>(aK0, aK1, klo[0], khi[0]);
@@ -1060,7 +985,7 @@
         } else {                                                                                        \
             lgkm_wait2<0>(klo[(i) % 4], khi[(i) % 4]);                                                  \
         }                                                                                               \
-        dq[dc_] = MFMA16(kc2_ ? dsf1 : dsf0, tr16_join8(klo[(i) % 4], khi[(i) % 4]), dq[dc_]);          \
+        dq[dc_] = MFMA16(tr16_join8(klo[(i) % 4], khi[(i) % 4]), dsf[kc2_], dq[dc_]);                   \
     }
             DQ_STEP(0) DQ_STEP(1) DQ_STEP(2) DQ_STEP(3)
             DQ_STEP(4) DQ_STEP(5) DQ_STEP(6) DQ_STEP(7)
@@ -1071,15 +996,14 @@
         }
     }
 
+    __bf16* dqrow = dqkv_q + (int64_t)(s0 + (qvalid ? qrow : 0)) * q_ts + q_hoff;
 #pragma unroll
     for (int dc = 0; dc < DCH; ++dc) {
-#pragma unroll
-        for (int r = 0; r < 4; ++r) {
-            const int qpos = qs + wave * 16 + lg * 4 + r;
-            const int d = dc * 16 + lr;
-            if (qpos < L && d < D)
-                dqkv_q[(int64_t)(s0 + qpos) * q_ts + q_hoff + d] = (__bf16)dq[dc][r];
-        }
+        const int d0 = dc * 16 + lg * 4;
+        bf16x4 dv;
+#pragma unroll
+        for (int x = 0; x < 4; ++x) dv[x] = (__bf16)dq[dc][x];
+        if (qvalid && d0 < D) *(bf16x4*)&dqrow[d0] = dv;
     }
 }
 
@@ -1091,7 +1015,6 @@
                          int64_t q_ts, int64_t q_gs, int64_t k_ts, int64_t k_hs,
                          int64_t v_ts, int64_t v_hs, int64_t do_ts, int max_tiles, float scale,
                          float p_drop, uint64_t seed) {
-    constexpr int ST = 64 + 8;
     dim3 block(512);
     dim3 grid(max_tiles, batch, H);
     constexpr int SQ = DPAD + 16;
@@ -1105,8 +1028,7 @@
                        seed_lo, seed_hi, thr, rp);
     int err = dol_last_error();
     if (err) return err;
-    size_t shmem_dq = (size_t)(64 * SQ * 2 + 8 * 16 * ST) * sizeof(__bf16);
-    hipLaunchKernelGGL((fa_bwd_dq_kernel<DPAD, DROPOUT>), grid, block, shmem_dq, stream,
+    hipLaunchKernelGGL((fa_bwd_dq_kernel<DPAD, DROPOUT>), grid, block, FaKvLds<DPAD>::bytes(DROPOUT), stream,
                        q, k, v, dout, lse, delta, dqkv_q, cu, H, Hkv, D, G,
                        q_ts, q_gs, k_ts, k_hs, v_ts, v_hs, do_ts, T, scale,
                        seed_lo, seed_hi, thr, rp);
diff --git a/tools_lds_sim.py b/tools_lds_sim.py
--- a/tools_lds_sim.py
+++ b/tools_lds_sim.py
@@ -134,6 +134,52 @@
     tot = [0, 0]
     print("  (patterns identical to dkv rows, SV=SK strides)")
 
+    regfrag_images()
+
+
+def PI23(q):
+    return (q & ~12) | (((q >> 2) & 1) << 3) | (((q >> 3) & 1) << 2)
+
+
+def read_tr16(addrs):
+    return cycles(addrs, G32, 2, 64)
+
+
+def regfrag_images():
+    print("== fa_fwd / fa_bwd_dq K,V images, register-resident P/dS ==")
+    for DPAD in (32, 64, 96, 128):
+        S = DPAD + 16
+        for place_name, place in (("natural", lambda r: r), ("PI23", PI23)):
+            wr = []
+            for base in range(0, 64 * DPAD // 8, 64):
+                addrs = {}
+                for l in range(64):
+                    pidx = base + l
+                    key, d0 = pidx // (DPAD // 8), (pidx % (DPAD // 8)) * 8
+                    addrs[l] = (place(key) * S + d0) * 2
+                wr.append(write128(addrs))
+            rd = []
+            for cb in range(4):
+                for kc in range(DPAD // 32):
+                    addrs = {}
+                    for l in range(64):
+                        lr, lg = lane_split(l)
+                        addrs[l] = (place(cb * 16 + lr) * S + kc * 32 + lg * 8) * 2
+                    rd.append(read128(addrs))
+            tr = []
+            for c in range(2):
+                for dc in range(DPAD // 16):
+                    for h in range(2):
+                        addrs = {}
+                        for l in range(64):
+                            row = 32 * c + 16 * h + 4 * (l >> 4) + ((l >> 2) & 3)
+                            addrs[l] = (place(row) * S + dc * 16 + 4 * (l & 3)) * 2
+                        tr.append(read_tr16(addrs))
+            print(f" DPAD={DPAD} stride={S} rows={place_name}")
+            report("staging b128 writes", wr)
+            report("b128 row reads (S^T / dP^T A-frags)", rd)
+            report("tr16 permuted-key reads (V^T / K^T A-frags)", tr)
+
 
 if __name__ == "__main__":
     main()
```

New measurement: 49330 tokens/s (median of 6 runs). +3.2%, better.
